# succinctlabs/sp1

Measured on AMD Instinct MI355X. Metric: RISC-V cycles proved/sec (core shard prove): whole ShardProof of a full core shard of the reference's `fibonacci` guest, see config, higher is better.
Workload: dtype u32 (KoalaBear Montgomery words, exact integer arithmetic)

## Files before the change

### __graft_entry__.py

```python
import os
import subprocess
import sys

ROOT = os.path.dirname(os.path.abspath(__file__))
CSRC = os.path.join(ROOT, "sp1_amd", "csrc")
LIB = os.path.join(ROOT, "sp1_amd", "lib", "libsp1hip.so")
HIP_SOURCES = ["runtime.hip", "merkle.hip", "ntt.hip", "ntt_fast.hip", "basefold.hip", "prover.hip", "stacked.hip", "zerocheck.hip", "zc_compile.cpp", "jagged.hip", "gkr.hip", "shard.hip", "staging.hip", "tracegen.hip", "tracegen_global.hip", "tracegen_riscv.hip", "tracegen_riscv_mem.hip", "tracegen_riscv_core.hip", "tracegen_riscv_sys.hip", "tracegen_rv64_partition.hip", "tracegen_lookup.hip", "tracegen_keccak.hip", "tracegen_weierstrass.hip", "host_par.hip", "pool.hip", "babybear.hip", "p2_host.cpp", "gkr_host.cpp", "rv64_exec.cpp", "outer.hip", "outer_host.cpp", "outer_basefold.hip", "outer_jagged.hip"]


def _stale(target, deps):
    if not os.path.exists(target):
        return True
    t = os.path.getmtime(target)
    return any(os.path.getmtime(d) > t for d in deps if os.path.exists(d))


def build_hip(force=False):
    from concurrent.futures import ThreadPoolExecutor
    srcs = [os.path.join(CSRC, s) for s in HIP_SOURCES if os.path.exists(os.path.join(CSRC, s))]
    headers = [os.path.join(CSRC, f) for f in os.listdir(CSRC) if f.endswith((".hpp", ".inc"))]
    headers.append(os.path.join(ROOT, "include", "sp1hip.h"))
    objdir = os.path.join(ROOT, "sp1_amd", "lib", "obj")
    os.makedirs(objdir, exist_ok=True)
    flags = ["--offload-arch=gfx950", "-O3", "-std=c++17", "-fPIC", "-Wall", "-Wno-unused-function", "-Wno-pass-failed"]
    extra = {"zerocheck.hip": ["-mllvm", "-pragma-unroll-threshold=1000000"]}
    objs, jobs = [], []
    for src in srcs:
        obj = os.path.join(objdir, os.path.basename(src)[:-4] + ".o")
        objs.append(obj)
        if force or _stale(obj, [src] + headers):
            jobs.append(["hipcc"] + (flags if src.endswith(".hip") else flags[1:]) + extra.get(os.path.basename(src), []) + ["-c", src, "-o", obj])
    if jobs:
        with ThreadPoolExecutor(max_workers=min(len(jobs), os.cpu_count() or 1)) as ex:
            list(ex.map(lambda cmd: subprocess.check_call(cmd, cwd=ROOT), jobs))
    if jobs or force or _stale(LIB, objs):
        subprocess.check_call(["hipcc", "--offload-arch=gfx950", "-shared", "-fPIC"] + objs + ["-lpthread", "-ldl", "-o", LIB], cwd=ROOT)
    build_native_tests()
    return LIB


def build_oracle(force=False):
    sys.path.insert(0, os.path.join(ROOT, "oracle"))
    import pyoracle
    return pyoracle.build(force)


def build_native_tests():
    exes = []
    for name, deps in (("rs_finish_stress", ["round_sync.hpp", "kb31.hpp", "common.hpp"]),
                       ("bn254_ops", ["bn254.hpp", "outer_poseidon2_rc.inc"]),
                       ("kb31_ops", ["kb31.hpp"]),
                       ("bb31_ops", ["bb31.hpp", "bb_poseidon2_rc.inc"]),
                       ("secp_rows", ["fp256.hpp", "tg_field_op.hpp", "kb31.hpp"]),
                       ("riscv_rows", ["tg_riscv_rows.hpp", "kb31.hpp", os.path.join(ROOT, "include", "sp1hip.h")]),
                       ("riscv_mem_rows", ["tg_riscv_mem_rows.hpp", "tg_riscv_rows.hpp", "kb31.hpp", os.path.join(ROOT, "include", "sp1hip.h")]),
                       ("riscv_core_rows", ["tg_riscv_core_rows.hpp", "tg_riscv_rows.hpp", "kb31.hpp", os.path.join(ROOT, "include", "sp1hip.h")]),
                       ("riscv_sys_rows", ["tg_riscv_sys_rows.hpp", "tg_rv64_partition.hpp", "tg_riscv_core_rows.hpp", "tg_riscv_rows.hpp", "kb31.hpp",
                                           os.path.join(ROOT, "include", "sp1hip.h")]),
                       ("lookup_counts", ["tg_lookup_counts.hpp", "kb31.hpp", os.path.join(ROOT, "include", "sp1hip.h")]),
                       ("septic_ops", ["septic.hpp", "poseidon2.hpp", "kb_poseidon2_rc.inc", "kb31.hpp"])):
        src = os.path.join(ROOT, "tests", "native", name + ".hip")
        exe = src[:-4]
        if not os.path.exists(src):
            continue
        if _stale(exe, [src] + [os.path.join(CSRC, d) for d in deps]):
            subprocess.check_call(["hipcc", "--offload-arch=gfx950", "-O3", "-std=c++17", "-I" + CSRC, "-I" + os.path.join(ROOT, "include"),
                                   src, "-ldl", "-o", exe], cwd=ROOT)
        exes.append(exe)
    return exes


def build():
    build_hip()
    build_oracle()
    sys.path.insert(0, ROOT)
    import sp1_amd
    lib = sp1_amd._lib.load()
    assert lib.sp1hip_version().startswith(b"sp1hip")
    subprocess.check_call([sys.executable, os.path.join(ROOT, "rust", "gen_sys.py")], stdout=subprocess.DEVNULL)


def smoke():
    sys.path.insert(0, ROOT)
    sys.path.insert(0, os.path.join(ROOT, "oracle"))
    import numpy as np
    import torch
    assert torch.cuda.is_available(), "smoke() needs a GPU"
    torch.cuda.set_device(0)
    import pyoracle as orc
    from sp1_amd import api

    lg_n, widths = 12, [16, 8]
    mles = [orc.random_felts((1 << lg_n, w), seed=7 + i) for i, w in enumerate(widths)]
    o_round = orc.CommittedRound(mles, 2)
    o_ch = orc.Challenger()
    o_ch.observe(o_round.commit)
    o_point = o_ch.sample_point(lg_n)
    o_claims = [orc.eval_mle(m, o_point) for m in mles]
    o_blob = orc.basefold_prove(o_point, [o_round], [o_claims], o_ch, 2, 16, 8)
    prover = api.BasefoldProver(2, 16, 8)
    d_mles = [api.ColMajor.from_row_major_host(m) for m in mles]
    commit, pd = prover.commit_mles(d_mles)
    assert np.array_equal(commit, o_round.commit), "commitment mismatch vs oracle"
    ch = api.DuplexChallenger()
    ch.observe(commit)
    point = ch.sample_point(lg_n)
    assert np.array_equal(point, o_point)
    claims = prover.evaluate_mles(d_mles, point)
    assert np.array_equal(claims, np.concatenate(o_claims)), "evaluation claims mismatch vs oracle"
    blob = prover.prove_trusted_mle_evaluations(point, [pd], claims, ch)
    assert blob == o_blob, "BaseFold proof bytes differ from the oracle"
    v_ch = orc.Challenger()
    v_ch.observe(commit)
    v_ch.sample_point(lg_n)
    assert orc.basefold_verify([commit], point, [claims], blob, v_ch, 2, 16, 8) == 0
    sys.path.insert(0, os.path.join(ROOT, "tests"))
    from shard_chips import make_shard_chips, preprocessed_round
    L, lsh, batch = 4, 3, 3
    chips, publics = make_shard_chips(5, 24, True, 3)
    o_prep = preprocessed_round(chips, L, lsh, batch, 1)
    jp = api.JaggedProver(L, lsh, batch, 1)
    dev = [(a, i, api.ColMajor.from_row_major_host(m) if m.shape[0] else None,
            api.ColMajor.from_row_major_host(p) if p is not None and p.shape[0] else None) for a, i, m, p in chips]
    g_commit, g_prep = jp.commit_multilinears([d[3] for d in dev if d[3] is not None])
    o_ch, g_ch = orc.Challenger(), api.DuplexChallenger()
    o_ch.observe(o_prep.commit)
    g_ch.observe(g_commit)
    v_ch = o_ch.clone()
    want = orc.shard_prove(chips, publics, o_prep, L, lsh, batch, o_ch, 1, 5, 4)
    got = api.prove_shard(dev, publics, g_prep, L, lsh, batch, g_ch, 1, 5, 4)
    assert got == want, "shard proof bytes differ from the oracle"
    assert orc.shard_verify(chips, g_commit, got, L, lsh, v_ch, 1, 5, 4) == 0
    sys.path.insert(0, os.path.join(ROOT, "bench"))
    import core_real
    from sp1_amd.machines import riscv_trace as RT
    counts = {"Add": 3, "Addi": 5, "Sub": 2, "Bitwise": 3, "Lt": 3, "Mul": 3, "ShiftLeft": 3, "ShiftRight": 3, "UType": 8,
              "LoadWord": 3, "LoadDouble": 3, "StoreWord": 3, "StoreDouble": 3, "Branch": 5, "Jal": 2, "Jalr": 2}
    machine, tabs, rpub = RT.generate(counts, K=2, seed=11, device="cuda")
    rpv = RT.to_monty_np(rpub)
    host = [(a, i, RT.to_monty_np(tabs[a.name][1]), RT.to_monty_np(tabs[a.name][0]) if tabs[a.name][0] is not None else None)
            for a, i in machine]
    rdev = [(a, i, core_real.to_col_major(tabs[a.name][1]), core_real.to_col_major(tabs[a.name][0]) if tabs[a.name][0] is not None else None)
            for a, i in machine]
    L, lsh, batch = 17, 12, 8
    r_prep = orc.JaggedRound([c[3] for c in host if c[3] is not None], L, lsh, batch, 1)
    rg_commit, rg_prep = api.JaggedProver(L, lsh, batch, 1).commit_multilinears([d[3] for d in rdev if d[3] is not None])
    assert np.array_equal(rg_commit, r_prep.commit), "RISC-V machine: preprocessed commitment differs from the oracle"
    o_ch, g_ch = orc.Challenger(), api.DuplexChallenger()
    o_ch.observe(r_prep.commit)
    g_ch.observe(rg_commit)
    orc.set_gkr_sparse(True)
    try:
        r_want = orc.shard_prove(host, rpv, r_prep, L, lsh, batch, o_ch, 1, 5, 4)
    finally:
        orc.set_gkr_sparse(False)
    r_got = api.prove_shard(rdev, rpv, rg_prep, L, lsh, batch, g_ch, 1, 5, 4)
    assert r_got == r_want, "RISC-V machine: shard proof bytes differ from the oracle"
    from sp1_amd.machines import riscv_more_trace as MT
    kmachine, ktabs, kpub = MT.precompile_shard(2, seed=3, device="cuda")
    khost = [(a, i, RT.to_monty_np(ktabs[a.name][1].cpu()), RT.to_monty_np(ktabs[a.name][0].cpu()) if ktabs[a.name][0] is not None else None)
             for a, i in kmachine]
    kdev = [(a, i, core_real.to_col_major(ktabs[a.name][1]), core_real.to_col_major(ktabs[a.name][0]) if ktabs[a.name][0] is not None else None)
            for a, i in kmachine]
    k_prep = orc.JaggedRound([c[3] for c in khost if c[3] is not None], L, lsh, batch, 1)
    kg_commit, kg_prep = api.JaggedProver(L, lsh, batch, 1).commit_multilinears([d[3] for d in kdev if d[3] is not None])
    o_ch, g_ch = orc.Challenger(), api.DuplexChallenger()
    o_ch.observe(k_prep.commit)
    g_ch.observe(kg_commit)
    publics = RT.to_monty_np(kpub.cpu())
    orc.set_gkr_sparse(True)
    try:
        k_want = orc.shard_prove(khost, publics, k_prep, L, lsh, batch, o_ch, 1, 5, 4)
    finally:
        orc.set_gkr_sparse(False)
    k_got = api.prove_shard(kdev, publics, kg_prep, L, lsh, batch, g_ch, 1, 5, 4)
    assert k_got == k_want, "Keccak precompile shard: proof bytes differ from the oracle"
    import struct
    from sp1_amd.machines import riscv_exec as RX
    ex = RX.Executor(RX.guest_file("fibonacci.elf"), stdin=[struct.pack("<Q", 20)])
    shard = ex.run_shard(1 << 20)
    assert shard.halted and shard.exit_code == 0, "the fibonacci guest did not halt cleanly"
    fmachine, ftabs, fpub = RX.shard_tables(ex, shard, device="cuda")
    fhost = [(a, i, RT.to_monty_np(ftabs[a.name][1]), RT.to_monty_np(ftabs[a.name][0]) if ftabs[a.name][0] is not None else None)
             for a, i in fmachine]
    fdev = [(a, i, core_real.to_col_major(ftabs[a.name][1]), core_real.to_col_major(ftabs[a.name][0]) if ftabs[a.name][0] is not None else None)
            for a, i in fmachine]
    fpv = RT.to_monty_np(fpub)
    f_prep = orc.JaggedRound([c[3] for c in fhost if c[3] is not None], L, lsh, batch, 1)
    fg_commit, fg_prep = api.JaggedProver(L, lsh, batch, 1).commit_multilinears([d[3] for d in fdev if d[3] is not None])
    o_ch, g_ch = orc.Challenger(), api.DuplexChallenger()
    o_ch.observe(f_prep.commit)
    g_ch.observe(fg_commit)
    orc.set_gkr_sparse(True)
    try:
        f_want = orc.shard_prove(fhost, fpv, f_prep, L, lsh, batch, o_ch, 1, 5, 4)
    finally:
        orc.set_gkr_sparse(False)
    f_got = api.prove_shard(fdev, fpv, fg_prep, L, lsh, batch, g_ch, 1, 5, 4)
    assert f_got == f_want, "fibonacci guest: shard proof bytes differ from the oracle"
    from sp1_amd.machines import public_values as PVM
    assert frozenset(a.name for a, _ in fmachine) in RT.chip_clusters(), "fibonacci guest: the shard is not a shape cluster"
    v_ch = orc.Challenger()
    v_ch.observe(f_prep.commit)
    shapes = [(a, i, np.zeros((0, a.main_width), np.uint32), np.zeros((0, a.prep_width), np.uint32) if a.prep_width else None) for a, i in fmachine]
    assert orc.shard_verify(shapes, fg_commit, f_got, L, lsh, v_ch, 1, 5, 4, pv_program=PVM.verifier_program()) == 0, \
        "fibonacci guest: the pinned verifier rejects the shard proof"
    torch.cuda.synchronize()
    print("smoke OK: commitment, claims, %d-byte BaseFold proof, %d-byte whole shard proof, a %d-byte proof of the rv64im machine "
          "(%d chips), a %d-byte proof of a Keccak precompile shard and a %d-byte proof of the reference's fibonacci guest "
          "(%d cycles) bit-identical to the oracle"
          % (len(blob), len(got), len(r_got), len(machine), len(k_got), len(f_got), shard.cycles))


if __name__ == "__main__":
    build()
    if len(sys.argv) > 1 and sys.argv[1] == "smoke":
        smoke()
```

### sp1_amd/csrc/gkr.hip

```cpp
#include <algorithm>
#include <array>
#include <chrono>
#include <cstring>
#include <optional>
#include <string>
#include <vector>

#include "device_ctx.hpp"
#include "host_par.hpp"

namespace sp1hip {
bool gkr_host_simd_available();
void gkr_host_round_sums(const uint32_t* tab, size_t stride, const uint32_t* eq, size_t eq_stride, size_t real_pairs, uint32_t out[6][4]);
void gkr_host_round_fold(const uint32_t* tab, uint32_t* out, size_t stride, size_t real_pairs, const uint32_t alpha[4]);
}
#include "round_sync.hpp"
#include "tensor_table.hpp"
#include "ext_host.hpp"
#include "gkr_kernels.hpp"

namespace sp1hip {

void challenger_observe(sp1hip_challenger_t* ch, uint32_t x);
kb::Ext challenger_sample_ext(sp1hip_challenger_t* ch);
void challenger_restore(sp1hip_challenger_t* dst, const sp1hip_challenger_t* src);

namespace gkr {

using namespace ext_host;

using Poly4 = std::array<Ext, 4>;
Ext poly_eval(const Poly4& c, const Ext& x) { return ((c[3] * x + c[2]) * x + c[1]) * x + c[0]; }

Poly4 interpolate4(const Ext (&xs)[4], const Ext (&ys)[4]) {
    Poly4 res{kb::ext_zero(), kb::ext_zero(), kb::ext_zero(), kb::ext_zero()};
    Ext num[4][4], den[4];
    bool live[4];
    for (int i = 0; i < 4; i++) {
        live[i] = !kb::ext_eq(ys[i], kb::ext_zero());
        if (!live[i]) continue;
        den[i] = kb::ext_one();
        Ext cur[4] = {ys[i], kb::ext_zero(), kb::ext_zero(), kb::ext_zero()};
        int deg = 0;
        for (int j = 0; j < 4; j++) {
            if (j == i) continue;
            den[i] = den[i] * (xs[i] - xs[j]);
            Ext nxt[4] = {kb::ext_zero(), kb::ext_zero(), kb::ext_zero(), kb::ext_zero()};
            for (int k = 0; k <= deg; k++) { nxt[k + 1] = nxt[k + 1] + cur[k]; nxt[k] = nxt[k] - cur[k] * xs[j]; }
            deg++;
            for (int k = 0; k < 4; k++) cur[k] = nxt[k];
        }
        for (int k = 0; k < 4; k++) num[i][k] = cur[k];
    }
    Ext prefix[4], running = kb::ext_one();
    for (int i = 0; i < 4; i++) if (live[i]) { prefix[i] = running; running = running * den[i]; }
    Ext inv_all = kb::ext_inv(running);
    for (int i = 3; i >= 0; i--) {
        if (!live[i]) continue;
        const Ext inv = inv_all * prefix[i];
        inv_all = inv_all * den[i];
        for (int k = 0; k < 4; k++) res[k] = res[k] + num[i][k] * inv;
    }
    return res;
}

struct Bytes {
    std::vector<uint8_t> b;
    void u64(uint64_t v) { for (int i = 0; i < 8; i++) b.push_back((uint8_t)(v >> (8 * i))); }
    void felt(uint32_t m) { const uint32_t v = kb::from_monty(m); for (int i = 0; i < 4; i++) b.push_back((uint8_t)(v >> (8 * i))); }
    void ext(const Ext& e) { for (int k = 0; k < 4; k++) felt(e.c[k]); }
};

void observe_ext(sp1hip_challenger_t* ch, const Ext& e) { for (int k = 0; k < 4; k++) challenger_observe(ch, e.c[k]); }

struct ChipInfo {
    std::string name;
    uint32_t rows, k, main_w, prep_w, int0;
    const uint32_t* d_main;
    const uint32_t* d_prep;
};

constexpr uint32_t MAX_TILES = 512;
uint32_t tiles_for(uint64_t threads) { return (uint32_t)std::min<uint64_t>(std::max<uint64_t>((threads + 255) / 256, 1), MAX_TILES); }

struct ParsedInt { uint32_t is_send, kind; std::vector<uint32_t> mult; std::vector<std::vector<uint32_t>> values; };
struct RoundOut { Ext n0, n1, d0, d1; std::vector<Poly4> polys; Ext claimed_sum, eval; std::vector<Ext> point; };
struct PassShape { int fv, sv; bool first; uint32_t tiles, tile_size, total_slots; size_t flat_off; bool flat; };

struct GkrTimer {
    enum Part { ROWS, INT, LAYER_HEAD, WAIT, HOST, LAUNCH, SKIP };
    using Clock = std::chrono::steady_clock;
    bool on = false;
    Clock::time_point last, clk[2];
    double part_ms[7] = {};
    int waits = 0;
    static double ms(Clock::time_point a, Clock::time_point b) { return std::chrono::duration<double, std::milli>(b - a).count(); }
    void start() { static const bool env = env_flag("SP1HIP_GKR_DEBUG", false); on = env; last = Clock::now(); }
    void mark(const char* what) {
        if (!on) return;
        const auto now = Clock::now();
        fprintf(stderr, "[sp1hip gkr] %-28s %8.3f ms\n", what, ms(last, now));
        last = now;
    }
    void lap(Part p) {
        if (!on) return;
        const auto now = Clock::now();
        part_ms[p] += ms(clk[p >= WAIT], now);
        clk[p >= WAIT] = now;
        waits += p == WAIT;
    }
    void report_layers() {
        if (!on) return;
        fprintf(stderr, "[sp1hip gkr]   of which row-variable rounds %.3f ms, interaction-variable rounds (host) %.3f ms\n", part_ms[ROWS], part_ms[INT]);
        fprintf(stderr, "[sp1hip gkr]   %d hand-overs inside the layers: waiting for the sums %.3f ms, closed forms + transcript %.3f ms, launch calls %.3f ms\n",
                waits, part_ms[WAIT], part_ms[HOST], part_ms[LAUNCH]);
    }
};

struct Levels {
    int L = 0;
    uint32_t K = 0;
    std::vector<uint32_t> h;
    std::vector<size_t> entries;
    std::vector<std::vector<size_t>> off;
    std::vector<DeviceBuf> N, D;
    uint32_t rows_at(uint32_t i, int l) const { return (uint32_t)(((uint64_t)h[i] + (((uint64_t)1 << (L - l)) - 1)) >> (L - l)); }
    void* n_ptr(int l, uint32_t i) const { return (char*)N[l].p + off[l][i] * (l == L ? 4 : 16); }
    Ext* d_ptr(int l, uint32_t i) const { return D[l].ext() + off[l][i]; }
    int alloc(int L_, std::vector<uint32_t> rows_of_interaction, hipStream_t s) {
        L = L_; h = std::move(rows_of_interaction); K = (uint32_t)h.size();
        entries.assign(L + 2, 0);
        off.assign(L + 1, std::vector<size_t>(K + 1, 0));
        for (int l = 1; l <= L; l++) {
            for (uint32_t i = 0; i < K; i++) off[l][i + 1] = off[l][i] + rows_at(i, l);
            entries[l] = off[l][K];
        }
        N = std::vector<DeviceBuf>(L + 1); D = std::vector<DeviceBuf>(L + 1);
        for (int l = 1; l <= L; l++) {
            SP1HIP_TRY(N[l].alloc(std::max<size_t>(entries[l], 1) * (l == L ? 4 : 16), s));
            SP1HIP_TRY(D[l].alloc(std::max<size_t>(entries[l], 1) * 16, s));
        }
        return SP1HIP_SUCCESS;
    }
};

struct PassPlan {
    std::vector<PassShape> shapes;
    std::vector<PassDesc> all_descs;
    std::vector<uint16_t> flat_index;
};
size_t count_passes(int L) { size_t n = 0; for (int v = 1; v <= L - 1; v++) n += (size_t)(v + 1) / 2 + 1; return n; }

void plan_passes(const Levels& lv, uint32_t flat_max_slots, Ext* const (&scratch)[2], Ext* host_rows, PassPlan& plan) {
    const uint32_t K = lv.K;
    auto scratch_ptr = [&](int b, uint32_t i, int which, const std::vector<size_t>& so) -> Ext* { return scratch[b] + 4 * so[i] + (size_t)which * (so[i + 1] - so[i]); };
    constexpr uint32_t TARGET_TILES = 2048;
    plan.all_descs.reserve(count_passes(lv.L) * K);
    std::vector<uint32_t> rows_in(K);
    std::vector<size_t> so_prev, so_next;
    for (int v = 1; v <= lv.L - 1; v++) {
        for (uint32_t i = 0; i < K; i++) rows_in[i] = (lv.rows_at(i, v + 1) + 1) / 2;
        int cur = 0, t = v, fv = 0, pass = 0;
        for (;;) {
            const int sv = std::min(2, t - fv);
            const bool first = pass <= 1;
            if (fv > 0) { so_next.assign(K + 1, 0); for (uint32_t i = 0; i < K; i++) so_next[i + 1] = so_next[i] + ((rows_in[i] + (1u << fv) - 1) >> fv); }
            uint64_t total_slots = 0;
            auto slots_of = [&](uint32_t rin) -> uint32_t { const uint32_t ro = (rin + (1u << fv) - 1) >> fv; return ((ro + (1u << sv) - 1) >> sv) << sv; };
            for (uint32_t i = 0; i < K; i++) total_slots += slots_of(rows_in[i]);
            const bool flat = total_slots <= flat_max_slots && K <= 65536;
            const uint32_t tile_size = flat ? 1u : (uint32_t)std::max<uint64_t>(256, ((total_slots + TARGET_TILES - 1) / TARGET_TILES + 255) / 256 * 256);
            const size_t flat_off = plan.flat_index.size();
            plan.all_descs.resize(plan.all_descs.size() + K);
            PassDesc* out = plan.all_descs.data() + plan.all_descs.size() - K;
            uint32_t tile0 = 0;
            for (uint32_t i = 0; i < K; i++) {
                PassDesc& d = out[i];
                d = PassDesc{};
                d.rows_in = rows_in[i]; d.eq_int_index = i;
                if (first) { d.src[0] = lv.n_ptr(v + 1, i); d.src[1] = lv.d_ptr(v + 1, i); d.rows_x = lv.rows_at(i, v + 1); }
                else for (int w = 0; w < 4; w++) d.src[w] = scratch_ptr(cur ^ 1, i, w, so_prev);
                if (fv > 0) for (int w = 0; w < 4; w++)
                    d.dst[w] = (sv == 0 && host_rows) ? host_rows + 4 * so_next[i] + (size_t)w * (so_next[i + 1] - so_next[i]) : scratch_ptr(cur, i, w, so_next);
                d.tile0 = tile0;
                const uint32_t n_tiles = (slots_of(rows_in[i]) + tile_size - 1) / tile_size;
                if (flat) plan.flat_index.insert(plan.flat_index.end(), n_tiles, (uint16_t)i);
                tile0 += n_tiles;
            }
            if (flat) plan.shapes.push_back(PassShape{fv, sv, first, std::max<uint32_t>((tile0 + 255) / 256, 1), tile_size, tile0, flat_off, true});
            else plan.shapes.push_back(PassShape{fv, sv, first, std::max<uint32_t>(tile0, 1), tile_size, tile0, 0, false});
            if (fv > 0) { for (uint32_t i = 0; i < K; i++) rows_in[i] = (rows_in[i] + (1u << fv) - 1) >> fv; so_prev = so_next; cur ^= 1; }
            t -= fv;
            pass++;
            if (sv == 0) break;
            fv = sv;
        }
    }
    if (plan.flat_index.empty()) plan.flat_index.push_back(0);
    plan.flat_index.resize((plan.flat_index.size() + 1) / 2 * 2);
}

struct Consts { const Ext one = kb::ext_one(), zero = kb::ext_zero(), inv8 = kb::ext_inv(ext_c(8)), inv2 = kb::ext_inv(ext_c(2)), four = ext_c(4); };

struct LayerRounds {
    sp1hip_challenger_t* ch;
    RoundOut ro;
    std::vector<Ext> alphas;
    Ext claim;
    Ext finish_round(const Poly4& poly, const Ext& pt, Ext& eq_factor) {
        ro.polys.push_back(poly);
        for (auto& c : poly) observe_ext(ch, c);
        const Ext a = challenger_sample_ext(ch), one = kb::ext_one();
        alphas.push_back(a);
        claim = poly_eval(poly, a);
        eq_factor = eq_factor * (pt * a + (one - pt) * (one - a));
        return a;
    }
};

Poly4 eq_times_quadratic(const Ext& scale, const Ext& pt, const Ext (&q)[3]) {
    const Ext e0 = scale * (kb::ext_one() - pt), e1 = scale * (pt + pt - kb::ext_one());
    return Poly4{e0 * q[0], e0 * q[1] + e1 * q[0], e0 * q[2] + e1 * q[1], e1 * q[2]};
}
void quadratic(const Ext& g0, const Ext& g1, const Ext& gi, Ext (&q)[3]) { q[0] = g0; q[1] = g1 - g0 - gi; q[2] = gi; }
Ext eval_quadratic(const Ext (&q)[3], const Ext& x) { return (q[2] * x + q[1]) * x + q[0]; }

void row_rounds_closed_form(int sv, const Ext (&S)[10], const std::vector<Ext>& row_point, int t, Ext& PA, LayerRounds& lr, Ext& a0, Ext& a1) {
    const Ext one = kb::ext_one(), pt_a = row_point[t - 1];
    if (sv == 2) {
        const Ext pt_b = row_point[t - 2];
        const Ext corr = one - S[9];
        Ext c0[3], c1[3], ci[3];
        quadratic(S[0] + corr, S[1] + corr, S[4], c0);
        quadratic(S[2] + corr, S[3] + corr, S[5], c1);
        quadratic(S[6], S[7], S[8], ci);
        Ext h[3];
        for (int k = 0; k < 3; k++) h[k] = c0[k] + pt_b * (c1[k] - c0[k]);
        a0 = lr.finish_round(eq_times_quadratic(PA, pt_a, h), pt_a, PA);
        const Ext g0 = eval_quadratic(c0, a0), g1 = eval_quadratic(c1, a0), gi = eval_quadratic(ci, a0);
        Ext gy[3];
        quadratic(g0, g1, gi, gy);
        a1 = lr.finish_round(eq_times_quadratic(PA, pt_b, gy), pt_b, PA);
    } else {
        const Ext corr = one - S[3];
        Ext h[3];
        quadratic(S[0] + corr, S[1] + corr, S[2], h);
        a0 = lr.finish_round(eq_times_quadratic(PA, pt_a, h), pt_a, PA);
        a1 = kb::ext_zero();
    }
}

constexpr size_t plane_stride(size_t n) { return ((n + 15) / 16) * 16 + 16; }

struct EqTabs {
    std::vector<std::vector<Ext>> tabs;
    std::vector<std::vector<uint32_t>> soa;
    void build(const std::vector<Ext>& int_point, bool simd) {
        const int niv = (int)int_point.size();
        tabs.assign(niv + 1, {}); soa.assign(niv + 1, {});
        tabs[0] = {kb::ext_one()};
        for (int m = 0; m < niv; m++) {
            const std::vector<Ext>& ev = tabs[m];
            std::vector<Ext>& nx = tabs[m + 1];
            nx.resize(ev.size() * 2);
            const Ext x = int_point[m];
            for (size_t i = 0; i < ev.size(); i++) { const Ext pr = ev[i] * x; nx[2 * i] = ev[i] - pr; nx[2 * i + 1] = pr; }
        }
        if (!simd) return;
        for (int m = 1; m <= niv; m++) {
            const size_t es = plane_stride((size_t)1 << m);
            soa[m].assign(4 * es, 0u);
            for (size_t i = 0; i < tabs[m].size(); i++)
                for (int k = 0; k < 4; k++) soa[m][(size_t)k * es + i] = tabs[m][i].c[k];
        }
    }
};

struct alignas(64) RoundSums { Ext x0, y0, xh, yh, e0, es; };

struct PlaneTables {
    const EqTabs& eq;
    const size_t stride;
    std::vector<uint32_t> soa[2];
    int side = 0;
    PlaneTables(const EqTabs& eq_, uint32_t W) : eq(eq_), stride(plane_stride(W)) {
        for (int b = 0; b < 2; b++) {
            soa[b].assign(16 * stride, 0u);
            for (int w = 1; w < 4; w += 2) std::fill_n(soa[b].begin() + (size_t)(4 * w) * stride, stride, kb::R1);
        }
    }
    void set_row(uint32_t i, const Ext* row) { for (int q = 0; q < 16; q++) soa[0][(size_t)q * stride + i] = row[q / 4].c[q % 4]; }
    RoundSums sums(int m, size_t real_pairs) const {
        uint32_t o6[6][4];
        gkr_host_round_sums(soa[side].data(), stride, eq.soa[m].data(), plane_stride((size_t)1 << m), real_pairs, o6);
        RoundSums t;
        Ext* dstp[6] = {&t.x0, &t.y0, &t.xh, &t.yh, &t.e0, &t.es};
        for (int q = 0; q < 6; q++) memcpy(dstp[q]->c, o6[q], 16);
        return t;
    }
    void fold(size_t real_pairs, size_t half, const Ext& alpha) {
        gkr_host_round_fold(soa[side].data(), soa[side ^ 1].data(), stride, real_pairs, alpha.c);
        if (real_pairs < half)
            for (int w = 0; w < 4; w++)
                for (int k = 0; k < 4; k++) soa[side ^ 1][(size_t)(4 * w + k) * stride + real_pairs] = (w & 1) && k == 0 ? kb::R1 : 0u;
        side ^= 1;
    }
    void first_row(Ext (&f)[4]) const { for (int q = 0; q < 16; q++) f[q / 4].c[q % 4] = soa[side][(size_t)q * stride]; }
};

struct ScalarTables {
    const EqTabs& eq;
    HostPar::Scope& par;
    std::vector<Ext> tab[2][4];
    int side = 0;
    ScalarTables(const EqTabs& eq_, HostPar::Scope& par_, uint32_t W) : eq(eq_), par(par_) {
        for (int w = 0; w < 4; w++) { tab[0][w].assign(W, (w & 1) ? kb::ext_one() : kb::ext_zero()); tab[1][w].resize(W / 2 + 1); }
    }
    void set_row(uint32_t i, const Ext* row) { for (int w = 0; w < 4; w++) tab[0][w][i] = row[w]; }
    RoundSums sums(int m, size_t real_pairs) const {
        const std::vector<Ext>& eqi = eq.tabs[m];
        const Ext *n0 = tab[side][0].data(), *d0 = tab[side][1].data(), *n1 = tab[side][2].data(), *d1 = tab[side][3].data();
        RoundSums parts[HostPar::Scope::MAX_THREADS];
        const int nparts = par.threads();
        for (int q = 0; q < nparts; q++) parts[q] = RoundSums{kb::ext_zero(), kb::ext_zero(), kb::ext_zero(), kb::ext_zero(), kb::ext_zero(), kb::ext_zero()};
        par.run(real_pairs, 24, [&](int part, size_t kb0, size_t ke) {
            RoundSums acc = parts[part];
            for (size_t k = kb0; k < ke; k++) {
                const size_t a = 2 * k, b = 2 * k + 1;
                acc.x0 = acc.x0 + eqi[a] * (d0[a] * n1[a] + d1[a] * n0[a]);
                acc.y0 = acc.y0 + eqi[a] * (d0[a] * d1[a]);
                const Ext sn0 = n0[a] + n0[b], sn1 = n1[a] + n1[b], sd0 = d0[a] + d0[b], sd1 = d1[a] + d1[b];
                const Ext es = eqi[a] + eqi[b];
                acc.xh = acc.xh + es * (sd0 * sn1 + sd1 * sn0);
                acc.yh = acc.yh + es * (sd0 * sd1);
                acc.e0 = acc.e0 + eqi[a];
                acc.es = acc.es + es;
            }
            parts[part] = acc;
        });
        RoundSums t = parts[0];
        for (int q = 1; q < nparts; q++) {
            t.x0 = t.x0 + parts[q].x0; t.y0 = t.y0 + parts[q].y0; t.xh = t.xh + parts[q].xh; t.yh = t.yh + parts[q].yh;
            t.e0 = t.e0 + parts[q].e0; t.es = t.es + parts[q].es;
        }
        return t;
    }
    void fold(size_t real_pairs, size_t half, const Ext& alpha) {
        const Ext *n0 = tab[side][0].data(), *d0 = tab[side][1].data(), *n1 = tab[side][2].data(), *d1 = tab[side][3].data();
        Ext *o0 = tab[side ^ 1][0].data(), *o1 = tab[side ^ 1][1].data(), *o2 = tab[side ^ 1][2].data(), *o3 = tab[side ^ 1][3].data();
        par.run(real_pairs, 48, [&](int, size_t kb0, size_t ke) {
            for (size_t k = kb0; k < ke; k++) {
                o0[k] = n0[2 * k] + alpha * (n0[2 * k + 1] - n0[2 * k]); o1[k] = d0[2 * k] + alpha * (d0[2 * k + 1] - d0[2 * k]);
                o2[k] = n1[2 * k] + alpha * (n1[2 * k + 1] - n1[2 * k]); o3[k] = d1[2 * k] + alpha * (d1[2 * k + 1] - d1[2 * k]);
            }
        });
        if (real_pairs < half) { o0[real_pairs] = kb::ext_zero(); o1[real_pairs] = kb::ext_one(); o2[real_pairs] = kb::ext_zero(); o3[real_pairs] = kb::ext_one(); }
        side ^= 1;
    }
    void first_row(Ext (&f)[4]) const { for (int w = 0; w < 4; w++) f[w] = tab[side][w][0]; }
};

template <class Tables>
void interaction_rounds(Tables& tb, size_t real, const std::vector<Ext>& int_point, const Ext& lambda, const Ext& PA, const Consts& k, LayerRounds& lr) {
    const int niv = (int)int_point.size();
    Ext eq_scale = k.one;
    for (int j = 0; j < niv; j++) {
        const size_t half = ((size_t)1 << (niv - j)) / 2, real_pairs = (real + 1) / 2;
        const RoundSums t = tb.sums(niv - j, real_pairs);
        const Ext pt = int_point[niv - 1 - j];
        const Ext s0 = lambda * t.x0 + t.y0 + ((k.one - pt) - t.e0);
        const Ext sh = lambda * t.xh + t.yh + (k.one - t.es) * k.four;
        const Ext PAe = PA * eq_scale;
        const Ext p0 = PAe * s0, ph = PAe * sh * k.inv8;
        const Ext xs[4] = {k.zero, k.one, k.inv2, (k.one - pt) * kb::ext_inv(k.one - (pt + pt))};
        const Ext ys[4] = {p0, lr.claim - p0, ph, k.zero};
        tb.fold(real_pairs, half, lr.finish_round(interpolate4(xs, ys), pt, eq_scale));
        real = real_pairs;
    }
    Ext f[4];
    tb.first_row(f);
    lr.ro.n0 = f[0]; lr.ro.d0 = f[1]; lr.ro.n1 = f[2]; lr.ro.d1 = f[3];
}

void interaction_rounds_host(bool simd, HostPar::Scope& par, const EqTabs& eq, uint32_t W, const std::vector<size_t>& so, const Ext* rows,
                             const std::vector<Ext>& int_point, const Ext& lambda, const Ext& PA, const Consts& k, LayerRounds& lr, GkrTimer& timer) {
    auto run = [&](auto tb) {
        const uint32_t K = (uint32_t)so.size() - 1;
        for (uint32_t i = 0; i < K; i++) if (so[i + 1] != so[i]) tb.set_row(i, rows + 4 * so[i]);
        timer.lap(GkrTimer::ROWS);
        interaction_rounds(tb, K, int_point, lambda, PA, k, lr);
        timer.lap(GkrTimer::INT);
    };
    if (simd) run(PlaneTables(eq, W)); else run(ScalarTables(eq, par, W));
}

#define SP1HIP_GKR_REQUIRE(cond, msg) \
    do { if (!(cond)) { sp1hip::set_error("sp1hip_logup_gkr_prove: %s", msg); return SP1HIP_ERROR_INVALID_ARGUMENT; } } while (0)

struct GkrProver {
    const sp1hip_gkr_chip_t* const chips;
    const int n_chips, L;
    sp1hip_challenger_t* const challenger;
    uint8_t* const h_proof;
    size_t* const proof_len;
    const sp1hip_stream_t stream;
    const hipStream_t s;

    GkrTimer timer;
    const Consts k;
    std::vector<ChipInfo> info;
    std::vector<ParsedInt> progs;
    size_t max_arity = 0, total_cols = 0, need = 0;
    uint32_t K = 0, W = 0;
    int niv = 0;
    struct Cloned { sp1hip_challenger_t* c = nullptr; ~Cloned() { sp1hip_challenger_free(c); } } clone;
    sp1hip_challenger_t* ch = nullptr;
    uint32_t witness = 0, flat_max_slots = 0;
    Ext alpha;
    std::vector<Ext> betas;
    std::vector<uint32_t> int_chip;
    Levels lv;
    size_t n_passes_total = 0;
    hipStream_t side = nullptr;
    hipEvent_t* side_ev = nullptr;
    DeviceBuf d_all, d_flat;
    PinnedStage side_stage, stage;
    DeviceBuf d_progs, d_betas, d_descs;
    std::vector<uint32_t> flat;
    std::vector<IntDesc> descs;
    DeviceBuf d_trans, d_trans2;
    Mailbox mb;
    DeviceBuf d_eq_int, d_T, d_TL, d_partials, scratch[2];
    bool direct_final = false, simd = false;
    PassPlan plan;
    std::vector<Ext> out_n, out_d, eval_point;
    Ext num_eval, den_eval;
    size_t launch_idx = 0;
    RoundSyncHost rsync;
    std::optional<HostPar::Scope> par;
    std::vector<RoundOut> rounds;
    std::vector<Ext> trace_point, openings;

    int parse_programs() {
        info.resize(n_chips);
        for (int c = 0; c < n_chips; c++) {
            const sp1hip_gkr_chip_t& ci = chips[c];
            SP1HIP_GKR_REQUIRE(ci.name && ci.interactions, "null chip field");
            SP1HIP_GKR_REQUIRE(ci.real_rows <= ((uint64_t)1 << L), "chip taller than 2^max_log_row_count");
            SP1HIP_GKR_REQUIRE(ci.real_rows == 0 || ci.main_width == 0 || ci.d_main, "null main trace");
            SP1HIP_GKR_REQUIRE(ci.real_rows == 0 || ci.prep_width == 0 || ci.d_prep, "null preprocessed trace");
            if (c) SP1HIP_GKR_REQUIRE(strcmp(chips[c - 1].name, ci.name) < 0, "chips must be sorted by name (BTreeSet order)");
            info[c] = ChipInfo{ci.name, (uint32_t)ci.real_rows, 0, ci.main_width, ci.prep_width, (uint32_t)progs.size(), ci.d_main, ci.d_prep};
            const uint32_t* p = ci.interactions;
            const uint32_t* end = p + ci.n_words;
            SP1HIP_GKR_REQUIRE(ci.n_words >= 1, "empty interaction program");
            const uint32_t ni = *p++;
            info[c].k = ni;
            auto vcol = [&](std::vector<uint32_t>& out) -> bool {
                if (p + 2 > end) return false;
                const uint32_t nt = p[0];
                if (p[1] >= kb::P || p + 2 + 3 * (size_t)nt > end) return false;
                out.push_back(nt);
                out.push_back(kb::to_monty(p[1]));
                p += 2;
                for (uint32_t t = 0; t < nt; t++, p += 3) {
                    if (p[0] > 1 || p[2] >= kb::P) return false;
                    if (p[1] >= (p[0] ? ci.main_width : ci.prep_width)) return false;
                    out.push_back(p[0]); out.push_back(p[1]); out.push_back(kb::to_monty(p[2]));
                }
                return true;
            };
            for (uint32_t i = 0; i < ni; i++) {
                SP1HIP_GKR_REQUIRE(p + 3 <= end, "truncated interaction program");
                const uint32_t nv = p[2];
                SP1HIP_GKR_REQUIRE(p[0] <= 1 && p[1] < kb::P && nv < 4096, "bad interaction header");
                ParsedInt pi{p[0], p[1], {}, std::vector<std::vector<uint32_t>>(nv)};
                p += 3;
                SP1HIP_GKR_REQUIRE(vcol(pi.mult), "bad multiplicity column");
                for (uint32_t j = 0; j < nv; j++) SP1HIP_GKR_REQUIRE(vcol(pi.values[j]), "bad value column (index or weight out of range)");
                max_arity = std::max<size_t>(max_arity, nv + 1);
                progs.push_back(std::move(pi));
            }
            SP1HIP_GKR_REQUIRE(p == end, "trailing words in interaction program");
            total_cols += (size_t)ci.main_width + ci.prep_width;
        }
        K = (uint32_t)progs.size();
        SP1HIP_GKR_REQUIRE(K >= 1, "no interactions in the shard");
        niv = log2_ceil(K);
        W = 1u << niv;
        return SP1HIP_SUCCESS;
    }

    size_t proof_size() const {
        size_t n = 2 * (8 + (size_t)2 * W * 16 + 24) + 8;
        for (int v = 1; v <= L - 1; v++) n += 64 + 8 + (size_t)(niv + v) * (8 + 64) + 16 + 8 + (size_t)(niv + v) * 16 + 16;
        n += 8 + (size_t)L * 16 + 8;
        for (int c = 0; c < n_chips; c++) {
            n += 8 + info[c].name.size() + 8 + (size_t)info[c].main_w * 16 + 16 + 1;
            if (info[c].prep_w) n += 8 + (size_t)info[c].prep_w * 16 + 16;
        }
        return n + 4;
    }

    int transcript_head() {
        SP1HIP_TRY(sp1hip_challenger_clone(challenger, &clone.c));
        ch = clone.c;
        SP1HIP_TRY(sp1hip_challenger_grind(ch, 12, &witness, stream));
        alpha = challenger_sample_ext(ch);
        std::vector<Ext> beta_seed(log2_ceil(max_arity));
        for (auto& b : beta_seed) b = challenger_sample_ext(ch);
        (void)challenger_sample_ext(ch);
        betas = partial_lagrange_host(beta_seed);
        return SP1HIP_SUCCESS;
    }

    int alloc_levels_and_plan_buffers() {
        int_chip.resize(K);
        std::vector<uint32_t> rows(K);
        for (int c = 0; c < n_chips; c++) for (uint32_t i = 0; i < info[c].k; i++) { int_chip[info[c].int0 + i] = c; rows[info[c].int0 + i] = info[c].rows; }
        SP1HIP_TRY(lv.alloc(L, std::move(rows), s));
        timer.mark("parse + level buffers");
        flat_max_slots = (uint32_t)env_uint("SP1HIP_GKR_FLAT_SLOTS", 65536);
        n_passes_total = count_passes(L);
        SP1HIP_TRY(aux_stream_for(s, 2, &side, &side_ev));
        SP1HIP_TRY(d_all.alloc(std::max<size_t>(n_passes_total * K, 1) * sizeof(PassDesc), side));
        SP1HIP_TRY(d_flat.alloc((n_passes_total * (size_t)flat_max_slots + 4) * sizeof(uint16_t), side));
        SP1HIP_TRY(side_stage.init(side));
        return stage.init(s);
    }

    int build_first_layer_and_tree() {
        std::vector<size_t> poff(K);
        for (uint32_t i = 0; i < K; i++) {
            poff[i] = flat.size();
            const ParsedInt& pi = progs[i];
            Ext head = alpha + kb::ext_mul_base(betas[0], kb::to_monty(pi.kind));
            uint32_t live = 0;
            for (size_t j = 0; j < pi.values.size(); j++) {
                if (pi.values[j][0] == 0) head = head + kb::ext_mul_base(betas[1 + j], pi.values[j][1]);
                else live++;
            }
            flat.insert(flat.end(), {pi.is_send, live, head.c[0], head.c[1], head.c[2], head.c[3]});
            flat.insert(flat.end(), pi.mult.begin(), pi.mult.end());
            for (size_t j = 0; j < pi.values.size(); j++) {
                if (pi.values[j][0] == 0) continue;
                flat.push_back((uint32_t)(1 + j));
                flat.insert(flat.end(), pi.values[j].begin(), pi.values[j].end());
            }
        }
        SP1HIP_TRY(upload(d_progs, flat.data(), flat.size() * 4, s, stage));
        SP1HIP_TRY(upload(d_betas, betas.data(), betas.size() * 16, s, stage));
        uint32_t max_rows = 0;
        descs.resize(K);
        for (uint32_t i = 0; i < K; i++) {
            const ChipInfo& c = info[int_chip[i]];
            descs[i] = IntDesc{d_progs.u32() + poff[i], c.d_main, c.d_prep, c.rows, (uint32_t*)lv.n_ptr(L, i), lv.d_ptr(L, i)};
            max_rows = std::max(max_rows, c.rows);
        }
        const bool fused_tree = L >= 3 && env_flag("SP1HIP_GKR_FUSED", true);
        if (fused_tree) {
            std::vector<FirstDesc> fdescs(K);
            for (uint32_t i = 0; i < K; i++)
                fdescs[i] = FirstDesc{descs[i].prog, descs[i].main, descs[i].prep, descs[i].rows, descs[i].n_out, descs[i].d_out,
                                      (Ext*)lv.n_ptr(L - 1, i), lv.d_ptr(L - 1, i), (Ext*)lv.n_ptr(L - 2, i), lv.d_ptr(L - 2, i)};
            SP1HIP_TRY(upload(d_descs, fdescs.data(), fdescs.size() * sizeof(FirstDesc), s, stage));
            if (max_rows) {
                ScopedTimer t("gkr_first_layer", s);
                hipLaunchKernelGGL(first_layers_kernel, dim3(tiles_for((max_rows + 3) / 4), K), dim3(256), 0, s, (const FirstDesc*)d_descs.p,
                                   (const Ext*)d_betas.p);
                SP1HIP_LAUNCH_CHECK();
            }
        } else {
            SP1HIP_TRY(upload(d_descs, descs.data(), descs.size() * sizeof(IntDesc), s, stage));
            if (max_rows) {
                ScopedTimer t("gkr_first_layer", s);
                hipLaunchKernelGGL(first_layer_kernel, dim3(tiles_for(max_rows), K), dim3(256), 0, s, (const IntDesc*)d_descs.p,
                                   (const Ext*)d_betas.p);
                SP1HIP_LAUNCH_CHECK();
            }
        }
        timer.mark("first layer enqueued");
        const int top = fused_tree ? L - 2 : L;
        std::vector<Trans2Desc> t2;
        std::vector<TransDesc> t1;
        std::vector<uint32_t> t2_mr, t1_mr;
        std::vector<int> t1_level;
        int l = top;
        if (fused_tree)
            for (; l >= 3; l -= 2) {
                uint32_t mr = 0;
                for (uint32_t i = 0; i < K; i++) {
                    const uint32_t rin = lv.rows_at(i, l);
                    t2.push_back(Trans2Desc{(const Ext*)lv.n_ptr(l, i), lv.d_ptr(l, i), (Ext*)lv.n_ptr(l - 1, i), lv.d_ptr(l - 1, i), (Ext*)lv.n_ptr(l - 2, i), lv.d_ptr(l - 2, i), rin});
                    mr = std::max(mr, (rin + 3) / 4);
                }
                t2_mr.push_back(mr);
            }
        for (; l >= 2; l--) {
            uint32_t mr = 0;
            for (uint32_t i = 0; i < K; i++) {
                const uint32_t rin = lv.rows_at(i, l);
                t1.push_back(TransDesc{lv.n_ptr(l, i), lv.d_ptr(l, i), (Ext*)lv.n_ptr(l - 1, i), lv.d_ptr(l - 1, i), rin});
                mr = std::max(mr, (rin + 1) / 2);
            }
            t1_mr.push_back(mr);
            t1_level.push_back(l);
        }
        if (!t2.empty()) SP1HIP_TRY(upload(d_trans2, t2.data(), t2.size() * sizeof(Trans2Desc), s, stage));
        if (!t1.empty()) SP1HIP_TRY(upload(d_trans, t1.data(), t1.size() * sizeof(TransDesc), s, stage));
        for (size_t j = 0; j < t2_mr.size(); j++) {
            if (!t2_mr[j]) continue;
            ScopedTimer t("gkr_transition", s);
            hipLaunchKernelGGL(transition2_kernel, dim3(tiles_for(t2_mr[j]), K), dim3(256), 0, s, (const Trans2Desc*)d_trans2.p + j * K);
            SP1HIP_LAUNCH_CHECK();
        }
        for (size_t j = 0; j < t1_mr.size(); j++) {
            if (!t1_mr[j]) continue;
            const TransDesc* d_t = (const TransDesc*)d_trans.p + j * K;
            ScopedTimer t("gkr_transition", s);
            if (t1_level[j] == L) hipLaunchKernelGGL(transition_kernel<true>, dim3(tiles_for(t1_mr[j]), K), dim3(256), 0, s, d_t);
            else hipLaunchKernelGGL(transition_kernel<false>, dim3(tiles_for(t1_mr[j]), K), dim3(256), 0, s, d_t);
            SP1HIP_LAUNCH_CHECK();
        }
        timer.mark("tree enqueued");
        return SP1HIP_SUCCESS;
    }

    int plan_and_upload_passes() {
        SP1HIP_TRY(mb.init(s));
        SP1HIP_TRY(d_eq_int.alloc((size_t)W * 16, s));
        SP1HIP_TRY(d_T.alloc(((size_t)2 << std::max(L - 1, 1)) * 16, s));
        SP1HIP_TRY(d_TL.alloc(((size_t)2 << std::max(L - 1, 1)) * 16, s));
        size_t scratch_entries = 0;
        for (uint32_t i = 0; i < K; i++) scratch_entries += (lv.rows_at(i, L) + 3) / 4 + 1;
        for (int b = 0; b < 2; b++) SP1HIP_TRY(scratch[b].alloc(std::max<size_t>(scratch_entries, 1) * 64, s));
        direct_final = (size_t)K * 16 + 4 <= MAILBOX_WORDS;
        Ext* const scratch_ext[2] = {scratch[0].ext(), scratch[1].ext()};
        plan_passes(lv, flat_max_slots, scratch_ext, direct_final ? reinterpret_cast<Ext*>(mb.h_slot + 4) : nullptr, plan);
        {
            uint32_t max_tiles = 1;
            for (auto& sh : plan.shapes) max_tiles = std::max(max_tiles, sh.tiles);
            SP1HIP_TRY(d_partials.alloc((size_t)max_tiles * 160, s));
        }
        timer.mark("pass descriptors planned");
        SP1HIP_GKR_REQUIRE(plan.all_descs.size() == n_passes_total * K, "internal error: pass count");
        SP1HIP_TRY(side_stage.upload(d_all.p, plan.all_descs.data(), plan.all_descs.size() * sizeof(PassDesc)));
        SP1HIP_GKR_REQUIRE(plan.flat_index.size() * sizeof(uint16_t) <= d_flat.n, "internal error: flat index size");
        SP1HIP_TRY(side_stage.upload(d_flat.p, plan.flat_index.data(), plan.flat_index.size() * sizeof(uint16_t)));
        SP1HIP_HIP(hipEventRecord(side_ev[1], side));
        SP1HIP_HIP(hipStreamWaitEvent(s, side_ev[1], 0));
        timer.mark("pass descriptors uploaded");
        return SP1HIP_SUCCESS;
    }

    int fetch_circuit_output() {
        out_n.assign(2 * (size_t)W, kb::ext_zero()); out_d.assign(2 * (size_t)W, kb::ext_one());
        std::vector<Ext> hn(std::max<size_t>(lv.entries[1], 1)), hd(std::max<size_t>(lv.entries[1], 1));
        if (L >= 2) {
            SP1HIP_TRY(mb.fetch(lv.N[1].p, lv.entries[1] * 4, hn.data()));
        } else {
            std::vector<uint32_t> hb(std::max<size_t>(lv.entries[1], 1));
            SP1HIP_TRY(mb.fetch(lv.N[1].p, lv.entries[1], hb.data()));
            for (size_t e = 0; e < lv.entries[1]; e++) hn[e] = kb::ext_from_base(hb[e]);
        }
        SP1HIP_TRY(mb.fetch(lv.D[1].p, lv.entries[1] * 4, hd.data()));
        for (uint32_t i = 0; i < K; i++)
            for (uint32_t r = 0; r < lv.rows_at(i, 1); r++) { out_n[2 * i + r] = hn[lv.off[1][i] + r]; out_d[2 * i + r] = hd[lv.off[1][i] + r]; }
        timer.mark("circuit output fetched");
        challenger_observe(ch, kb::to_monty(2 * W));
        for (auto& e : out_n) observe_ext(ch, e);
        challenger_observe(ch, kb::to_monty(2 * W));
        for (auto& e : out_d) observe_ext(ch, e);
        eval_point.resize(niv + 1);
        for (auto& z : eval_point) z = challenger_sample_ext(ch);
        num_eval = eval_mle_host(out_n, eval_point); den_eval = eval_mle_host(out_d, eval_point);
        return SP1HIP_SUCCESS;
    }

#define SP1HIP_GKR_PASS(FV, SV, F, NB, FL) hipLaunchKernelGGL((gkr_pass<FV, SV, F, NB, FL>), dim3(shape.tiles), dim3(256), 0, s, d_descs, (const Ext*)d_eq_int.p, Tp, TLp, c0, c1, d_partials.u32(), rs, publish_rows ? mb.seq + 1 : rsync.seq, K, shape.tile_size, fa)
#define SP1HIP_GKR_PASS_FL(FV, SV, F, NB) do { if (shape.flat) SP1HIP_GKR_PASS(FV, SV, F, NB, true); else SP1HIP_GKR_PASS(FV, SV, F, NB, false); } while (0)
#define SP1HIP_GKR_PASS_SRC(FV, SV) do { if (nbase) SP1HIP_GKR_PASS_FL(FV, SV, true, true); else if (shape.first) SP1HIP_GKR_PASS_FL(FV, SV, true, false); else SP1HIP_GKR_PASS_FL(FV, SV, false, false); } while (0)
    int launch_pass(size_t idx, int v, int t_after, const Ext& c0, const Ext& c1) {
        const PassShape shape = plan.shapes[idx];
        const PassDesc* d_descs = (const PassDesc*)d_all.p + idx * K;
        const int fv = shape.fv, sv = shape.sv;
        const FlatArgs fa{(const uint16_t*)d_flat.p + shape.flat_off, shape.total_slots};
        const bool nbase = shape.first && v + 1 == L;
        const bool publish_rows = sv == 0 && direct_final;
        if (publish_rows) { rsync.pending = true; mb.pending = true; }
        const RoundSync rs = sv > 0 ? rsync.next() : publish_rows ? RoundSync{rsync.d_counter, (volatile uint32_t*)mb.h_slot} : RoundSync{};
        const Ext* Tp = sv > 0 ? d_T.ext() + (((size_t)1 << (t_after - sv)) - 1) : (const Ext*)nullptr;
        const Ext* TLp = sv > 0 ? d_TL.ext() + (((size_t)1 << (t_after - sv)) - 1) : (const Ext*)nullptr;
        ScopedTimer tm(fv == 0 ? "gkr_pass_sum" : sv == 0 ? "gkr_pass_fold" : "gkr_pass_fold_sum", s);
        if (fv == 0 && sv == 2) { if (nbase) SP1HIP_GKR_PASS_FL(0, 2, true, true); else SP1HIP_GKR_PASS_FL(0, 2, true, false); }
        else if (fv == 0 && sv == 1) { if (nbase) SP1HIP_GKR_PASS_FL(0, 1, true, true); else SP1HIP_GKR_PASS_FL(0, 1, true, false); }
        else if (fv == 2 && sv == 2) SP1HIP_GKR_PASS_SRC(2, 2);
        else if (fv == 2 && sv == 1) SP1HIP_GKR_PASS_SRC(2, 1);
        else if (fv == 2 && sv == 0) SP1HIP_GKR_PASS_SRC(2, 0);
        else if (fv == 1 && sv == 0) SP1HIP_GKR_PASS_SRC(1, 0);
        else { set_error("internal error: GKR pass shape (%d, %d)", fv, sv); return SP1HIP_ERROR_RUNTIME; }
        SP1HIP_LAUNCH_CHECK();
        return SP1HIP_SUCCESS;
    }
#undef SP1HIP_GKR_PASS_SRC
#undef SP1HIP_GKR_PASS_FL
#undef SP1HIP_GKR_PASS

    int prove_layer(int v) {
        timer.lap(GkrTimer::LAYER_HEAD);
        const Ext lambda = challenger_sample_ext(ch);
        LayerRounds lr{ch, {}, {}, num_eval * lambda + den_eval};
        lr.ro.claimed_sum = lr.claim;
        const std::vector<Ext> int_point(eval_point.begin(), eval_point.begin() + niv), row_point(eval_point.begin() + niv, eval_point.end());
        SP1HIP_GKR_REQUIRE(niv <= 32 && v <= 32, "point too long");
        {
            PointArg pi{}, pa{};
            for (int j = 0; j < niv; j++) pi.c[j] = int_point[j];
            for (int j = 0; j < v; j++) pa.c[j] = row_point[j];
            const uint32_t full_blocks = (W + 255) / 256, prefix_blocks = ((2u << v) + 255) / 256;
            hipLaunchKernelGGL(eq_layer_tables_kernel, dim3(full_blocks + prefix_blocks), dim3(256), 0, s, pi, niv, d_eq_int.ext(), full_blocks, pa, v,
                               lambda, d_T.ext(), d_TL.ext());
            SP1HIP_LAUNCH_CHECK();
        }
        EqTabs eq_tabs;
        Ext PA = k.one;
        Ext a0 = k.zero, a1 = k.zero;
        int t = v;
        for (bool first_pass = true;; first_pass = false) {
            const size_t idx = launch_idx++;
            const int fv = plan.shapes[idx].fv, sv = plan.shapes[idx].sv;
            t -= fv;
            if (!simd && t == sv) par->wake();
            timer.lap(first_pass ? GkrTimer::SKIP : GkrTimer::HOST);
            SP1HIP_TRY(launch_pass(idx, v, t, a0, a1));
            timer.lap(GkrTimer::LAUNCH);
            if (first_pass) eq_tabs.build(int_point, simd);
            if (sv == 0) break;
            const int ns = sv == 2 ? 10 : 4;
            uint32_t h_sums[40];
            timer.lap(GkrTimer::SKIP);
            SP1HIP_TRY(rsync.wait(h_sums, 4 * ns));
            timer.lap(GkrTimer::WAIT);
            Ext S[10];
            memcpy(S, h_sums, 16 * (size_t)ns);
            row_rounds_closed_form(sv, S, row_point, t, PA, lr, a0, a1);
        }
        std::vector<size_t> so(K + 1, 0);
        for (uint32_t i = 0; i < K; i++) so[i + 1] = so[i] + (lv.rows_at(i, v + 1) ? 1 : 0);
        const size_t final_rows_total = so[K];
        const int cur = (int)((((v + 1) / 2)) & 1) ^ 1;
        std::vector<Ext> host(std::max<size_t>(final_rows_total, 1) * 4);
        if (direct_final) { SP1HIP_TRY(mb.wait_next(host.data(), final_rows_total * 16, 4)); rsync.pending = false; }
        else SP1HIP_TRY(mb.fetch(scratch[cur].p, final_rows_total * 16, host.data()));
        interaction_rounds_host(simd, *par, eq_tabs, W, so, host.data(), int_point, lambda, PA, k, lr, timer);
        RoundOut& ro = lr.ro;
        ro.eval = lr.claim;
        ro.point.assign(lr.alphas.rbegin(), lr.alphas.rend());
        observe_ext(ch, ro.n0); observe_ext(ch, ro.n1); observe_ext(ch, ro.d0); observe_ext(ch, ro.d1);
        eval_point = ro.point;
        const Ext lc = challenger_sample_ext(ch);
        num_eval = ro.n0 + (ro.n1 - ro.n0) * lc;
        den_eval = ro.d0 + (ro.d1 - ro.d0) * lc;
        eval_point.push_back(lc);
        rounds.push_back(std::move(ro));
        par->park();
        return SP1HIP_SUCCESS;
    }

    int prove_layers() {
        SP1HIP_TRY(rsync.init(s));
        simd = gkr_host_simd_available();
        par.emplace();
        par->park();
        for (int v = 1; v <= L - 1; v++) SP1HIP_TRY(prove_layer(v));
        timer.report_layers();
        timer.mark("all layers");
        return SP1HIP_SUCCESS;
    }

    int open_traces() {
        trace_point.assign(eval_point.end() - L, eval_point.end());
        openings.assign(std::max<size_t>(total_cols, 1), kb::ext_zero());
        if (!total_cols) return SP1HIP_SUCCESS;
        DeviceBuf d_eq, d_od, d_part, d_res;
        SP1HIP_TRY(d_eq.alloc(((size_t)16) << L, s));
        SP1HIP_TRY(sp1hip_partial_lagrange(reinterpret_cast<const sp1hip_ext_t*>(trace_point.data()), L, d_eq.u32(), stream));
        std::vector<OpenDesc> od;
        uint32_t out0 = 0, max_rows_open = 0;
        for (int c = 0; c < n_chips; c++) {
            for (uint32_t g = 0; g < info[c].main_w; g += OPEN_COLS) od.push_back(OpenDesc{info[c].d_main, info[c].rows, info[c].main_w, g, out0 + g});
            out0 += info[c].main_w;
            for (uint32_t g = 0; g < info[c].prep_w; g += OPEN_COLS) od.push_back(OpenDesc{info[c].d_prep, info[c].rows, info[c].prep_w, g, out0 + g});
            out0 += info[c].prep_w;
            max_rows_open = std::max(max_rows_open, info[c].rows);
        }
        const uint32_t chunks = std::max<uint32_t>((max_rows_open + OPEN_ROWS - 1) / OPEN_ROWS, 1);
        SP1HIP_TRY(upload(d_od, od.data(), od.size() * sizeof(OpenDesc), s, stage));
        SP1HIP_TRY(d_part.alloc((size_t)chunks * total_cols * 16, s));
        SP1HIP_TRY(d_res.alloc(total_cols * 16, s));
        SP1HIP_HIP(hipMemsetAsync(d_part.p, 0, (size_t)chunks * total_cols * 16, s));
        ScopedTimer t("gkr_openings", s);
        hipLaunchKernelGGL(open_columns_kernel, dim3((uint32_t)od.size(), chunks), dim3(256), 0, s, (const OpenDesc*)d_od.p, d_eq.u32(),
                           1u << L, d_part.u32(), (uint32_t)total_cols);
        SP1HIP_LAUNCH_CHECK();
        hipLaunchKernelGGL(open_sum_kernel, dim3(((uint32_t)total_cols * 4 + 63) / 64), dim3(256), 0, s, d_part.u32(), chunks,
                           (uint32_t)total_cols * 4, d_res.u32());
        SP1HIP_LAUNCH_CHECK();
        return mb.fetch(d_res.p, total_cols * 4, openings.data());
    }

    void observe_openings() {
        challenger_observe(ch, kb::to_monty((uint32_t)n_chips));
        size_t o = 0;
        for (int c = 0; c < n_chips; c++) {
            const Ext* main = openings.data() + o;
            const Ext* prep = main + info[c].main_w;
            if (info[c].prep_w) {
                challenger_observe(ch, kb::to_monty(info[c].prep_w));
                for (uint32_t j = 0; j < info[c].prep_w; j++) observe_ext(ch, prep[j]);
            }
            challenger_observe(ch, kb::to_monty(info[c].main_w));
            for (uint32_t j = 0; j < info[c].main_w; j++) observe_ext(ch, main[j]);
            o += info[c].main_w + info[c].prep_w;
        }
        timer.mark("openings");
    }

    int write_proof() {
        Bytes w;
        for (const std::vector<Ext>* vv : {&out_n, &out_d}) {
            w.u64(vv->size());
            for (auto& e : *vv) w.ext(e);
            w.u64(2); w.u64(vv->size()); w.u64(1);
        }
        w.u64(rounds.size());
        for (auto& r : rounds) {
            w.ext(r.n0); w.ext(r.n1); w.ext(r.d0); w.ext(r.d1);
            w.u64(r.polys.size());
            for (auto& p : r.polys) { w.u64(4); for (auto& c : p) w.ext(c); }
            w.ext(r.claimed_sum);
            w.u64(r.point.size());
            for (auto& x : r.point) w.ext(x);
            w.ext(r.eval);
        }
        w.u64(trace_point.size());
        for (auto& x : trace_point) w.ext(x);
        w.u64(n_chips);
        size_t o = 0;
        for (int c = 0; c < n_chips; c++) {
            w.u64(info[c].name.size());
            for (char chr : info[c].name) w.b.push_back((uint8_t)chr);
            w.u64(info[c].main_w);
            for (uint32_t j = 0; j < info[c].main_w; j++) w.ext(openings[o + j]);
            w.u64(1); w.u64(info[c].main_w);
            w.b.push_back(info[c].prep_w ? 1 : 0);
            if (info[c].prep_w) {
                w.u64(info[c].prep_w);
                for (uint32_t j = 0; j < info[c].prep_w; j++) w.ext(openings[o + info[c].main_w + j]);
                w.u64(1); w.u64(info[c].prep_w);
            }
            o += info[c].main_w + info[c].prep_w;
        }
        w.felt(witness);
        if (w.b.size() != need) {
            set_error("internal error: GKR proof size %zu != expected %zu", w.b.size(), need);
            return SP1HIP_ERROR_RUNTIME;
        }
        memcpy(h_proof, w.b.data(), w.b.size());
        *proof_len = w.b.size();
        return SP1HIP_SUCCESS;
    }

    int prove() {
        timer.start();
        SP1HIP_TRY(parse_programs());
        need = proof_size();
        if (!h_proof || *proof_len < need) {
            *proof_len = need;
            set_error("sp1hip_logup_gkr_prove: proof buffer too small, need %zu bytes", need);
            return SP1HIP_ERROR_BUFFER_TOO_SMALL;
        }
        const DeviceCtx* ctx;
        SP1HIP_TRY(get_device_ctx(&ctx));
        SP1HIP_TRY(transcript_head());
        SP1HIP_TRY(alloc_levels_and_plan_buffers());
        SP1HIP_TRY(build_first_layer_and_tree());
        SP1HIP_TRY(plan_and_upload_passes());
        SP1HIP_TRY(fetch_circuit_output());
        SP1HIP_TRY(prove_layers());
        SP1HIP_TRY(open_traces());
        observe_openings();
        SP1HIP_TRY(write_proof());
        challenger_restore(challenger, ch);
        return SP1HIP_SUCCESS;
    }
};
#undef SP1HIP_GKR_REQUIRE
}
}

using namespace sp1hip;

extern "C" int sp1hip_logup_gkr_prove(const sp1hip_gkr_chip_t* chips, int n_chips, int max_log_row_count, sp1hip_challenger_t* challenger,
                                      uint8_t* h_proof, size_t* proof_len, sp1hip_stream_t stream) {
    SP1HIP_REQUIRE(chips && n_chips > 0 && challenger && proof_len, "bad argument");
    SP1HIP_REQUIRE(max_log_row_count >= 1 && max_log_row_count <= 30, "max_log_row_count out of range");
    gkr::GkrProver p{chips, n_chips, max_log_row_count, challenger, h_proof, proof_len, stream, S(stream)};
    return p.prove();
}
```

### sp1_amd/csrc/gkr_kernels.hpp

```cpp
#pragma once
#include "device_ctx.hpp"
#include "round_sync.hpp"

namespace sp1hip {
namespace gkr {

using Ext = kb::Ext;

__device__ __forceinline__ Ext ld_ext(const Ext* p, uint32_t i) {
    const q4_t v = gptr(reinterpret_cast<const q4_t*>(p))[i];
    return Ext{{v.x, v.y, v.z, v.w}};
}
__device__ __forceinline__ void st_ext(Ext* p, uint32_t i, const Ext& e) {
    const q4_t v = {e.c[0], e.c[1], e.c[2], e.c[3]};
    gptr(reinterpret_cast<q4_t*>(p))[i] = v;
}

__device__ __forceinline__ void st_ext_host(Ext* p, uint32_t i, const Ext& e) {
    uint32_t* w = reinterpret_cast<uint32_t*>(p + i);
#pragma unroll
    for (int k = 0; k < 4; k++) __hip_atomic_store(w + k, e.c[k], __ATOMIC_RELAXED, __HIP_MEMORY_SCOPE_SYSTEM);
}

__device__ __forceinline__ uint32_t wave_sum(uint32_t v) {
#pragma unroll
    for (int off = 32; off >= 1; off >>= 1) v = kb::add(v, __shfl_down(v, off, 64));
    return v;
}
template <int NS>
__device__ __forceinline__ void block_reduce_store(const Ext (&acc)[NS], uint32_t* out) {
    __shared__ uint32_t sm[4][4 * NS];
    const int lane = threadIdx.x & 63, wave = threadIdx.x >> 6;
#pragma unroll
    for (int s = 0; s < NS; s++)
#pragma unroll
        for (int k = 0; k < 4; k++) {
            const uint32_t w = wave_sum(acc[s].c[k]);
            if (lane == 0) sm[wave][4 * s + k] = w;
        }
    __syncthreads();
    if (threadIdx.x < 4 * NS) {
        uint32_t a = 0;
        for (int i = 0; i < 4; i++) a = kb::add(a, sm[i][threadIdx.x]);
        out[threadIdx.x] = a;
    }
}
template <int NS>
__global__ __launch_bounds__(256) void reduce_partials(const uint32_t* __restrict__ partials, uint32_t n, uint32_t* out) {
    Ext acc[NS];
#pragma unroll
    for (int s = 0; s < NS; s++) acc[s] = kb::ext_zero();
    for (uint32_t i = threadIdx.x; i < n; i += 256)
#pragma unroll
        for (int s = 0; s < NS; s++) {
            const uint32_t* q = partials + ((size_t)i * NS + s) * 4;
            acc[s] = kb::ext_add(acc[s], Ext{{q[0], q[1], q[2], q[3]}});
        }
    block_reduce_store<NS>(acc, out);
}

__device__ __forceinline__ uint32_t level_pos(uint32_t e, uint32_t len) {
    return (e | 511u) < len ? ((e & ~511u) | ((e & 7u) << 6) | ((e >> 3) & 63u)) : e;
}

struct IntDesc {
    const uint32_t* prog;
    const uint32_t* main;
    const uint32_t* prep;
    uint32_t rows;
    uint32_t* n_out;
    Ext* d_out;
};

typedef const uint32_t __attribute__((address_space(4)))* prog_words_t;
__device__ __forceinline__ uint32_t vcol_apply(prog_words_t& p, const IntDesc& d, uint32_t r) {
    const uint32_t nt = p[0];
    uint32_t acc = p[1];
    p += 2;
    for (uint32_t t = 0; t < nt; t++, p += 3) {
        const uint32_t* col = (p[0] ? d.main : d.prep) + (size_t)p[1] * d.rows;
        const uint32_t v = gptr(col)[r], wgt = p[2];
        acc = kb::add(acc, wgt == kb::R1 ? v : kb::mul(v, wgt));
    }
    return acc;
}

__global__ __launch_bounds__(256) void first_layer_kernel(const IntDesc* __restrict__ descs, const Ext* __restrict__ betas) {
    const IntDesc d = descs[blockIdx.y];
    for (uint32_t r = blockIdx.x * blockDim.x + threadIdx.x; r < d.rows; r += gridDim.x * blockDim.x) {
        prog_words_t p = (prog_words_t)(uintptr_t)d.prog;
        const bool is_send = p[0] != 0;
        const uint32_t nv = p[1];
        Ext den{{p[2], p[3], p[4], p[5]}};
        p += 6;
        uint32_t m = vcol_apply(p, d, r);
        if (!is_send) m = kb::sub(0u, m);
        for (uint32_t j = 0; j < nv; j++) {
            const uint32_t bi = *p++;
            den = kb::ext_add(den, kb::ext_mul_base(ld_ext(betas, bi), vcol_apply(p, d, r)));
        }
        const uint32_t rp = level_pos(r, d.rows);
        gptr(d.n_out)[rp] = m;
        st_ext(d.d_out, rp, den);
    }
}

struct TransDesc {
    const void* n_in;
    const Ext* d_in;
    Ext* n_out;
    Ext* d_out;
    uint32_t rows_in;
};

template <bool NBASE>
__device__ __forceinline__ Ext load_n(const void* p, uint32_t i) {
    if (NBASE) return kb::ext_from_base(gptr((const uint32_t*)p)[i]);
    return ld_ext((const Ext*)p, i);
}

template <bool NBASE>
__global__ __launch_bounds__(256) void transition_kernel(const TransDesc* __restrict__ descs) {
    const TransDesc d = descs[blockIdx.y];
    const uint32_t rows_out = (d.rows_in + 1) / 2;
    for (uint32_t r = blockIdx.x * blockDim.x + threadIdx.x; r < rows_out; r += gridDim.x * blockDim.x) {
        const uint32_t ia = level_pos(2 * r, d.rows_in), ib = level_pos(2 * r + 1, d.rows_in), io = level_pos(r, rows_out);
        const Ext da = ld_ext(d.d_in, ia);
        if (2 * r + 1 < d.rows_in) {
            const Ext db = ld_ext(d.d_in, ib);
            Ext n;
            if (NBASE) {
                const uint32_t na = gptr((const uint32_t*)d.n_in)[ia], nb = gptr((const uint32_t*)d.n_in)[ib];
                n = kb::ext_add(kb::ext_mul_base(db, na), kb::ext_mul_base(da, nb));
            } else {
                n = kb::ext_add(kb::ext_mul(db, load_n<false>(d.n_in, ia)), kb::ext_mul(da, load_n<false>(d.n_in, ib)));
            }
            st_ext(d.n_out, io, n);
            st_ext(d.d_out, io, kb::ext_mul(da, db));
        } else {
            st_ext(d.n_out, io, load_n<NBASE>(d.n_in, ia));
            st_ext(d.d_out, io, da);
        }
    }
}

struct FirstDesc {
    const uint32_t* prog;
    const uint32_t* main;
    const uint32_t* prep;
    uint32_t rows;
    uint32_t* n0_out;
    Ext* d0_out;
    Ext* n1_out; Ext* d1_out;
    Ext* n2_out; Ext* d2_out;
};

__device__ __forceinline__ void vcol_apply4(prog_words_t& p, const FirstDesc& d, uint32_t q, bool vec, uint32_t (&out)[4]) {
    const uint32_t nt = p[0], c0 = p[1];
    p += 2;
#pragma unroll
    for (int j = 0; j < 4; j++) out[j] = c0;
    for (uint32_t t = 0; t < nt; t++, p += 3) {
        const uint32_t* col = (p[0] ? d.main : d.prep) + (size_t)p[1] * d.rows;
        const uint32_t wgt = p[2];
        uint32_t v[4];
        if (vec) {
            const q4_t x = gptr(reinterpret_cast<const q4_t*>(col))[q];
            v[0] = x.x; v[1] = x.y; v[2] = x.z; v[3] = x.w;
        } else {
#pragma unroll
            for (int j = 0; j < 4; j++) v[j] = 4 * q + j < d.rows ? gptr(col)[4 * q + j] : 0u;
        }
#pragma unroll
        for (int j = 0; j < 4; j++) out[j] = kb::add(out[j], wgt == kb::R1 ? v[j] : kb::mul(v[j], wgt));
    }
}

__global__ __launch_bounds__(256) void first_layers_kernel(const FirstDesc* __restrict__ descs, const Ext* __restrict__ betas) {
    const FirstDesc d = descs[blockIdx.y];
    const uint32_t quads = (d.rows + 3) / 4, rows1 = (d.rows + 1) / 2, rows2 = (rows1 + 1) / 2;
    const bool vec = (d.rows & 3u) == 0;
    for (uint32_t q = blockIdx.x * blockDim.x + threadIdx.x; q < quads; q += gridDim.x * blockDim.x) {
        prog_words_t p = (prog_words_t)(uintptr_t)d.prog;
        const bool is_send = p[0] != 0;
        const uint32_t nv = p[1];
        const Ext head{{p[2], p[3], p[4], p[5]}};
        p += 6;
        uint32_t m[4], val[4];
        vcol_apply4(p, d, q, vec, m);
        Ext den[4];
#pragma unroll
        for (int j = 0; j < 4; j++) { if (!is_send) m[j] = kb::sub(0u, m[j]); den[j] = head; }
        uint64_t acc[4][4];
#pragma unroll
        for (int j = 0; j < 4; j++)
#pragma unroll
            for (int c = 0; c < 4; c++) acc[j][c] = 0;
        uint32_t pending = 0;
        for (uint32_t k = 0; k < nv; k++) {
            const uint32_t bi = *p++;
            vcol_apply4(p, d, q, vec, val);
            const Ext b = ld_ext(betas, bi);
#pragma unroll
            for (int j = 0; j < 4; j++)
#pragma unroll
                for (int c = 0; c < 4; c++) acc[j][c] += (uint64_t)b.c[c] * val[j];
            if (++pending == 4 || k + 1 == nv) {
#pragma unroll
                for (int j = 0; j < 4; j++)
#pragma unroll
                    for (int c = 0; c < 4; c++) { den[j].c[c] = kb::add(den[j].c[c], kb::monty_reduce_wide(acc[j][c])); acc[j][c] = 0; }
                pending = 0;
            }
        }
        const uint32_t live = min(4u, d.rows - 4 * q);
#pragma unroll
        for (int j = 0; j < 4; j++)
            if ((uint32_t)j < live) {
                const uint32_t rp = level_pos(4 * q + j, d.rows);
                gptr(d.n0_out)[rp] = m[j];
                st_ext(d.d0_out, rp, den[j]);
            }
        Ext n1[2], d1[2];
#pragma unroll
        for (int h = 0; h < 2; h++) {
            if ((uint32_t)(2 * h + 1) < live) {
                n1[h] = kb::ext_add(kb::ext_mul_base(den[2 * h + 1], m[2 * h]), kb::ext_mul_base(den[2 * h], m[2 * h + 1]));
                d1[h] = kb::ext_mul(den[2 * h], den[2 * h + 1]);
            } else { n1[h] = kb::ext_from_base(m[2 * h]); d1[h] = den[2 * h]; }
            if ((uint32_t)(2 * h) < live) {
                const uint32_t io = level_pos(2 * q + h, rows1);
                st_ext(d.n1_out, io, n1[h]); st_ext(d.d1_out, io, d1[h]);
            }
        }
        const uint32_t io = level_pos(q, rows2);
        if (live > 2) {
            st_ext(d.n2_out, io, kb::ext_add(kb::ext_mul(d1[1], n1[0]), kb::ext_mul(d1[0], n1[1])));
            st_ext(d.d2_out, io, kb::ext_mul(d1[0], d1[1]));
        } else { st_ext(d.n2_out, io, n1[0]); st_ext(d.d2_out, io, d1[0]); }
    }
}

struct Trans2Desc {
    const Ext* n_in; const Ext* d_in;
    Ext* n1_out; Ext* d1_out; Ext* n2_out; Ext* d2_out;
    uint32_t rows_in;
};
__global__ __launch_bounds__(256) void transition2_kernel(const Trans2Desc* __restrict__ descs) {
    const Trans2Desc d = descs[blockIdx.y];
    const uint32_t quads = (d.rows_in + 3) / 4, rows1 = (d.rows_in + 1) / 2, rows2 = (rows1 + 1) / 2;
    for (uint32_t q = blockIdx.x * blockDim.x + threadIdx.x; q < quads; q += gridDim.x * blockDim.x) {
        const uint32_t live = min(4u, d.rows_in - 4 * q);
        Ext n[4], dd[4];
#pragma unroll
        for (int j = 0; j < 4; j++)
            if ((uint32_t)j < live) { const uint32_t ip = level_pos(4 * q + j, d.rows_in); n[j] = ld_ext(d.n_in, ip); dd[j] = ld_ext(d.d_in, ip); }
        Ext n1[2], d1[2];
#pragma unroll
        for (int h = 0; h < 2; h++) {
            if ((uint32_t)(2 * h + 1) < live) {
                n1[h] = kb::ext_add(kb::ext_mul(dd[2 * h + 1], n[2 * h]), kb::ext_mul(dd[2 * h], n[2 * h + 1]));
                d1[h] = kb::ext_mul(dd[2 * h], dd[2 * h + 1]);
            } else if ((uint32_t)(2 * h) < live) { n1[h] = n[2 * h]; d1[h] = dd[2 * h]; }
            if ((uint32_t)(2 * h) < live) {
                const uint32_t io = level_pos(2 * q + h, rows1);
                st_ext(d.n1_out, io, n1[h]); st_ext(d.d1_out, io, d1[h]);
            }
        }
        const uint32_t io = level_pos(q, rows2);
        if (live > 2) {
            st_ext(d.n2_out, io, kb::ext_add(kb::ext_mul(d1[1], n1[0]), kb::ext_mul(d1[0], n1[1])));
            st_ext(d.d2_out, io, kb::ext_mul(d1[0], d1[1]));
        } else { st_ext(d.n2_out, io, n1[0]); st_ext(d.d2_out, io, d1[0]); }
    }
}

struct PointArg { Ext c[32]; };
__global__ __launch_bounds__(256) void eq_layer_tables_kernel(PointArg pi, int niv, Ext* __restrict__ eq_int, uint32_t full_blocks,
                                                              PointArg pa, int v, Ext lambda, Ext* __restrict__ T, Ext* __restrict__ TL) {
    if (blockIdx.x < full_blocks) {
        const uint32_t i = blockIdx.x * 256u + threadIdx.x;
        if (i >= (1u << niv)) return;
        Ext acc = kb::ext_one();
        for (int j = 0; j < niv; j++) {
            const bool bit = (i >> (niv - 1 - j)) & 1u;
            acc = kb::ext_mul(acc, bit ? pi.c[j] : kb::ext_sub(kb::ext_one(), pi.c[j]));
        }
        st_ext(eq_int, i, acc);
        return;
    }
    const uint32_t g = (blockIdx.x - full_blocks) * 256u + threadIdx.x + 1;
    if (g >= (2u << v)) return;
    const int t = 31 - __clz(g);
    const uint32_t i = g - (1u << t);
    Ext acc = kb::ext_one();
    for (int j = 0; j < t; j++) {
        const bool bit = (i >> (t - 1 - j)) & 1u;
        acc = kb::ext_mul(acc, bit ? pa.c[j] : kb::ext_sub(kb::ext_one(), pa.c[j]));
    }
    st_ext(T, g - 1, acc);
    st_ext(TL, g - 1, kb::ext_mul(acc, lambda));
}

struct PassDesc {
    const void* src[4];
    Ext* dst[4];
    uint32_t rows_in;
    uint32_t rows_x;
    uint32_t eq_int_index;
    uint32_t tile0;
};

__device__ __forceinline__ uint32_t find_desc(const PassDesc* __restrict__ descs, uint32_t K, uint32_t b) {
    uint32_t lo = 0, hi = K;
    while (hi - lo > 1) {
        const uint32_t mid = (lo + hi) >> 1;
        if (descs[mid].tile0 <= b) lo = mid; else hi = mid;
    }
    return lo;
}
struct Row { Ext n0, d0, n1, d1; };

__device__ __forceinline__ uint32_t folded_pos(uint32_t r, uint32_t len) {
    return (r | 255u) < len ? ((r & ~255u) | ((r & 3u) << 6) | ((r >> 2) & 63u)) : r;
}

__device__ __forceinline__ Row padding_row() { return Row{kb::ext_zero(), kb::ext_one(), kb::ext_zero(), kb::ext_one()}; }

template <bool FIRST, bool NBASE>
__device__ __forceinline__ Row load_row(const PassDesc& d, uint32_t r) {
    Row q = padding_row();
    if (r >= d.rows_in) return q;
    if (FIRST) {
        const uint32_t ea = level_pos(2 * r, d.rows_x), eb = level_pos(2 * r + 1, d.rows_x);
        q.n0 = load_n<NBASE>(d.src[0], ea);
        q.d0 = ld_ext((const Ext*)d.src[1], ea);
        if (2 * r + 1 < d.rows_x) { q.n1 = load_n<NBASE>(d.src[0], eb); q.d1 = ld_ext((const Ext*)d.src[1], eb); }
    } else {
        const uint32_t rp = folded_pos(r, d.rows_in);
        q.n0 = ld_ext((const Ext*)d.src[0], rp); q.d0 = ld_ext((const Ext*)d.src[1], rp);
        q.n1 = ld_ext((const Ext*)d.src[2], rp); q.d1 = ld_ext((const Ext*)d.src[3], rp);
    }
    return q;
}

__device__ __forceinline__ Ext lerp(const Ext& a, const Ext& b, const Ext& t) { return kb::ext_add(a, kb::ext_mul(kb::ext_sub(b, a), t)); }
__device__ __forceinline__ Row lerp_row(const Row& a, const Row& b, const Ext& t) {
    return Row{lerp(a.n0, b.n0, t), lerp(a.d0, b.d0, t), lerp(a.n1, b.n1, t), lerp(a.d1, b.d1, t)};
}
__device__ __forceinline__ Ext lerp_base(uint32_t a, uint32_t b, const Ext& t) {
    Ext e = kb::ext_mul_base(t, kb::sub(b, a));
    e.c[0] = kb::add(e.c[0], a);
    return e;
}
template <bool NBASE>
__device__ __forceinline__ Row lerp_row_in(const Row& a, const Row& b, const Ext& t) {
    if (!NBASE) return lerp_row(a, b, t);
    return Row{lerp_base(a.n0.c[0], b.n0.c[0], t), lerp(a.d0, b.d0, t), lerp_base(a.n1.c[0], b.n1.c[0], t), lerp(a.d1, b.d1, t)};
}

template <int FV, bool FIRST, bool NBASE>
__device__ __forceinline__ Row fold_row(const PassDesc& d, uint32_t ro, const Ext& a0, const Ext& a1) {
    if constexpr (FV == 0) return load_row<FIRST, NBASE>(d, ro);
    Row in[FV == 0 ? 1 : (1 << FV)];
#pragma unroll
    for (int j = 0; j < (1 << FV); j++) in[j] = load_row<FIRST, NBASE>(d, (ro << FV) + j);
    if constexpr (FV == 1) return lerp_row_in<NBASE>(in[0], in[1], a0);
    else {
        const Row lo = lerp_row_in<NBASE>(in[0], in[1], a0), hi = lerp_row_in<NBASE>(in[2], in[3], a0);
        return lerp_row(lo, hi, a1);
    }
}

template <int CTRL>
__device__ __forceinline__ Ext dpp_ext(const Ext& e) {
    return Ext{{p2::dpp_mov<CTRL>(e.c[0]), p2::dpp_mov<CTRL>(e.c[1]), p2::dpp_mov<CTRL>(e.c[2]), p2::dpp_mov<CTRL>(e.c[3])}};
}
__device__ __forceinline__ Ext sel_ext(bool c, const Ext& a, const Ext& b) {
    return Ext{{c ? a.c[0] : b.c[0], c ? a.c[1] : b.c[1], c ? a.c[2] : b.c[2], c ? a.c[3] : b.c[3]}};
}

template <int SV> struct GridAcc { Ext a[SV == 2 ? 5 : 3]; };
template <int SV>
__device__ __forceinline__ void grid_init(GridAcc<SV>& g) {
#pragma unroll
    for (int i = 0; i < (SV == 2 ? 5 : 3); i++) g.a[i] = kb::ext_zero();
}

template <int SV, bool NB>
__device__ __forceinline__ void grid_accumulate(const Row& row, const Ext& w, const Ext& wl, uint32_t j, GridAcc<SV>& g) {
    const Ext A = kb::ext_add(NB ? kb::ext_mul_base(wl, row.n0.c[0]) : kb::ext_mul(row.n0, wl), kb::ext_mul(row.d0, w));
    const Ext B = NB ? kb::ext_mul_base(wl, row.n1.c[0]) : kb::ext_mul(row.n1, wl);
    g.a[0] = kb::ext_add(g.a[0], kb::ext_add(kb::ext_mul(B, row.d0), kb::ext_mul(A, row.d1)));
    const bool lo1 = (j & 1u) == 0;
    const Ext P = sel_ext(lo1, B, A), Q = sel_ext(lo1, row.d0, row.d1), PS = sel_ext(lo1, A, B), QS = sel_ext(lo1, row.d1, row.d0);
    const Ext DP = kb::ext_sub(P, dpp_ext<p2::DPP_QUAD_SWAP1>(PS)), DQ = kb::ext_sub(Q, dpp_ext<p2::DPP_QUAD_SWAP1>(QS));
    g.a[1] = kb::ext_add(g.a[1], kb::ext_mul(DP, DQ));
    if constexpr (SV == 2) {
        const bool lo2 = (j & 2u) == 0;
        const Ext P2 = sel_ext(lo2, B, A), Q2 = sel_ext(lo2, row.d0, row.d1), PS2 = sel_ext(lo2, A, B), QS2 = sel_ext(lo2, row.d1, row.d0);
        const Ext EP = kb::ext_sub(P2, dpp_ext<p2::DPP_QUAD_SWAP2>(PS2)), EQ = kb::ext_sub(Q2, dpp_ext<p2::DPP_QUAD_SWAP2>(QS2));
        g.a[2] = kb::ext_add(g.a[2], kb::ext_mul(EP, EQ));
        const Ext FP = kb::ext_sub(DP, dpp_ext<p2::DPP_QUAD_SWAP2>(DP)), FQ = kb::ext_sub(DQ, dpp_ext<p2::DPP_QUAD_SWAP2>(DQ));
        g.a[3] = kb::ext_add(g.a[3], kb::ext_mul(FP, FQ));
    }
    if (j == 0) g.a[SV == 2 ? 4 : 2] = kb::ext_add(g.a[SV == 2 ? 4 : 2], w);
}

template <int SV> struct GridOut { static constexpr int NS = SV == 2 ? 10 : 4; };
template <int SV>
__device__ __forceinline__ void grid_split(const GridAcc<SV>& g, uint32_t j, const Ext& scale, bool use_scale, Ext (&out)[GridOut<SV>::NS]) {
    const Ext z = kb::ext_zero();
    Ext a[SV == 2 ? 5 : 3];
#pragma unroll
    for (int i = 0; i < (SV == 2 ? 5 : 3); i++) a[i] = use_scale ? kb::ext_mul(g.a[i], scale) : g.a[i];
    if constexpr (SV == 2) {
        out[0] = j == 0 ? a[0] : z; out[1] = j == 1 ? a[0] : z; out[2] = j == 2 ? a[0] : z; out[3] = j == 3 ? a[0] : z;
        out[4] = j < 2 ? a[1] : z; out[5] = j < 2 ? z : a[1];
        out[6] = (j & 1u) == 0 ? a[2] : z; out[7] = (j & 1u) == 0 ? z : a[2];
        out[8] = j < 2 ? a[3] : z;
        out[9] = a[4];
    } else {
        out[0] = j == 0 ? a[0] : z; out[1] = j == 1 ? a[0] : z;
        out[2] = a[1];
        out[3] = a[2];
    }
}

struct FlatArgs { const uint16_t* index; uint32_t total_slots; };

template <int FV, int SV, bool FIRST, bool NBASE, bool FLAT>
__global__ __launch_bounds__(256) void gkr_pass(const PassDesc* __restrict__ descs, const Ext* __restrict__ eq_int,
                                                const Ext* __restrict__ T, const Ext* __restrict__ TL, Ext a0, Ext a1,
                                                uint32_t* __restrict__ partials, RoundSync rs, uint32_t seq, uint32_t K,
                                                uint32_t tile_size, FlatArgs fa) {
    static_assert(FV + SV > 0 && FV <= 2 && SV <= 2, "a pass folds and / or sums");
    constexpr int SVS = SV == 0 ? 1 : SV;
    GridAcc<SVS> g;
    grid_init<SVS>(g);
    const uint32_t j = threadIdx.x & ((1u << SV) - 1u);
    auto do_row = [&](const PassDesc& d, uint32_t ro, bool valid, const Ext& wi, bool use_wi) {
        const uint32_t rows_out = (d.rows_in + (1u << FV) - 1u) >> FV;
        Row row = padding_row();
        if (valid && ro < rows_out) {
            row = fold_row<FV, FIRST, NBASE>(d, ro, a0, a1);
            if (FV > 0) {
                const uint32_t rq = folded_pos(ro, rows_out);
                if (SV == 0 && rs.host_slot != nullptr) {
                    st_ext_host(d.dst[0], rq, row.n0); st_ext_host(d.dst[1], rq, row.d0); st_ext_host(d.dst[2], rq, row.n1); st_ext_host(d.dst[3], rq, row.d1);
                } else {
                    st_ext(d.dst[0], rq, row.n0); st_ext(d.dst[1], rq, row.d0); st_ext(d.dst[2], rq, row.n1); st_ext(d.dst[3], rq, row.d1);
                }
            }
        }
        if constexpr (SV > 0) {
            const uint32_t cells = (rows_out + (1u << SV) - 1u) >> SV;
            const uint32_t c = ro >> SV;
            Ext w = kb::ext_zero(), wl = kb::ext_zero();
            if (valid && c < cells) {
                w = ld_ext(T, c); wl = ld_ext(TL, c);
                if (use_wi) { w = kb::ext_mul(w, wi); wl = kb::ext_mul(wl, wi); }
            }
            grid_accumulate<SVS, FIRST && NBASE && FV == 0>(row, w, wl, j, g);
        }
    };
    Ext scale = kb::ext_one();
    if (FLAT) {
        const uint32_t p = blockIdx.x * 256 + threadIdx.x;
        const bool valid = p < fa.total_slots;
        const PassDesc d = descs[valid ? fa.index[p] : 0];
        const Ext wi = SV > 0 ? ld_ext(eq_int, d.eq_int_index) : kb::ext_one();
        do_row(d, p - d.tile0, valid, wi, true);
    } else {
        const PassDesc d = descs[find_desc(descs, K, blockIdx.x)];
        const uint32_t rows_out = (d.rows_in + (1u << FV) - 1u) >> FV;
        const uint32_t slots = ((rows_out + (1u << SV) - 1u) >> SV) << SV;
        const uint32_t k0 = (blockIdx.x - d.tile0) * tile_size, k1 = min(slots, k0 + tile_size);
        for (uint32_t base = k0; base < k1; base += 256) do_row(d, base + threadIdx.x, base + threadIdx.x < k1, scale, false);
        if (SV > 0) scale = ld_ext(eq_int, d.eq_int_index);
    }
    if constexpr (SV > 0) {
        Ext out[GridOut<SVS>::NS];
        grid_split<SVS>(g, j, scale, !FLAT, out);
        rs_finish<GridOut<SVS>::NS>(out, partials, blockIdx.x, gridDim.x, rs, seq);
    } else if (rs.host_slot != nullptr) {
        asm volatile("s_waitcnt vmcnt(0)" ::: "memory");
        __syncthreads();
        if (threadIdx.x == 0 && rs_ticket_is_last_acq_rel(rs.counter, blockIdx.x, gridDim.x)) rs_publish_seq(rs.host_slot, seq);
    }
}

struct OpenDesc { const uint32_t* cols; uint32_t rows, width, col0, out0; };
constexpr int OPEN_COLS = 4, OPEN_ROWS = 16384;
__global__ __launch_bounds__(256) void open_columns_kernel(const OpenDesc* __restrict__ descs, const uint32_t* __restrict__ eq,
                                                           uint32_t eq_len, uint32_t* __restrict__ partials, uint32_t total_cols) {
    const OpenDesc d = descs[blockIdx.x];
    const uint32_t r0 = blockIdx.y * OPEN_ROWS;
    if (r0 >= d.rows) return;
    kb::DotAcc acc[OPEN_COLS];
#pragma unroll
    for (int c = 0; c < OPEN_COLS; c++) kb::dot_init(acc[c]);
    for (uint32_t r = r0 + threadIdx.x; r < r0 + OPEN_ROWS && r < d.rows; r += 256) {
        const Ext e{{eq[r], eq[eq_len + r], eq[2 * (size_t)eq_len + r], eq[3 * (size_t)eq_len + r]}};
#pragma unroll
        for (int c = 0; c < OPEN_COLS; c++)
            if (d.col0 + c < d.width) kb::dot_add(acc[c], e, gptr(d.cols)[(size_t)(d.col0 + c) * d.rows + r]);
    }
    __shared__ uint32_t sm[4][4 * OPEN_COLS];
    const int lane = threadIdx.x & 63, wave = threadIdx.x >> 6;
#pragma unroll
    for (int c = 0; c < OPEN_COLS; c++) {
        const Ext v = kb::dot_finish(acc[c]);
#pragma unroll
        for (int k = 0; k < 4; k++) {
            const uint32_t w = wave_sum(v.c[k]);
            if (lane == 0) sm[wave][4 * c + k] = w;
        }
    }
    __syncthreads();
    if (threadIdx.x < 4 * OPEN_COLS) {
        const int c = threadIdx.x / 4;
        if (d.col0 + c < d.width) {
            uint32_t a = 0;
            for (int i = 0; i < 4; i++) a = kb::add(a, sm[i][threadIdx.x]);
            partials[((size_t)blockIdx.y * total_cols + d.out0 + c) * 4 + (threadIdx.x & 3)] = a;
        }
    }
}
__global__ __launch_bounds__(256) void open_sum_kernel(const uint32_t* __restrict__ partials, uint32_t n_chunks, uint32_t n_words, uint32_t* __restrict__ out) {
    __shared__ uint32_t sm[256];
    const uint32_t jl = threadIdx.x & 63u, cl = threadIdx.x >> 6, j = blockIdx.x * 64u + jl;
    uint32_t acc = 0;
    if (j < n_words)
        for (uint32_t c = cl; c < n_chunks; c += 4) acc = kb::add(acc, partials[(size_t)c * n_words + j]);
    sm[threadIdx.x] = acc;
    __syncthreads();
    if (cl == 0 && j < n_words) out[j] = kb::add(kb::add(sm[jl], sm[64 + jl]), kb::add(sm[128 + jl], sm[192 + jl]));
}
}
}
```

### sp1_amd/csrc/round_sync.hpp

```cpp
#pragma once
#include <chrono>
#include <cstring>
#include <vector>
#include <algorithm>

#include "common.hpp"
#include "kb31.hpp"

#if defined(__HIP_DEVICE_COMPILE__) && !defined(__gfx950__) && !defined(__gfx942__)
#error "round_sync.hpp: the sc1 + vmcnt(0) hand-over is only valid on gfx942/gfx950"
#endif

namespace sp1hip {

struct RoundSync {
    uint32_t* counter;
    volatile uint32_t* host_slot;
};

constexpr uint32_t RS_GROUPS = 32, RS_GROUP_STRIDE = 64;
constexpr size_t RS_COUNTER_BYTES = (size_t)(RS_GROUPS + 1) * RS_GROUP_STRIDE * 4;
constexpr size_t RS_SLOT_WORDS = 64;

__device__ __forceinline__ bool rs_ticket_is_last(uint32_t* counter, uint32_t block_linear, uint32_t total_blocks) {
    const uint32_t g = block_linear % RS_GROUPS, members = (total_blocks - g + RS_GROUPS - 1) / RS_GROUPS;
    uint32_t* cg = counter + g * RS_GROUP_STRIDE;
    if (__hip_atomic_fetch_add(cg, 1u, __ATOMIC_RELAXED, __HIP_MEMORY_SCOPE_AGENT) != members - 1) return false;
    __hip_atomic_store(cg, 0u, __ATOMIC_RELAXED, __HIP_MEMORY_SCOPE_AGENT);
    uint32_t* c2 = counter + RS_GROUPS * RS_GROUP_STRIDE;
    const uint32_t groups = total_blocks < RS_GROUPS ? total_blocks : RS_GROUPS;
    if (__hip_atomic_fetch_add(c2, 1u, __ATOMIC_RELAXED, __HIP_MEMORY_SCOPE_AGENT) != groups - 1) return false;
    __hip_atomic_store(c2, 0u, __ATOMIC_RELAXED, __HIP_MEMORY_SCOPE_AGENT);
    return true;
}
__device__ __forceinline__ bool rs_ticket_is_last_acq_rel(uint32_t* counter, uint32_t block_linear, uint32_t total_blocks) {
    const uint32_t g = block_linear % RS_GROUPS, members = (total_blocks - g + RS_GROUPS - 1) / RS_GROUPS;
    uint32_t* cg = counter + g * RS_GROUP_STRIDE;
    if (__hip_atomic_fetch_add(cg, 1u, __ATOMIC_ACQ_REL, __HIP_MEMORY_SCOPE_AGENT) != members - 1) return false;
    __hip_atomic_store(cg, 0u, __ATOMIC_RELAXED, __HIP_MEMORY_SCOPE_AGENT);
    uint32_t* c2 = counter + RS_GROUPS * RS_GROUP_STRIDE;
    const uint32_t groups = total_blocks < RS_GROUPS ? total_blocks : RS_GROUPS;
    if (__hip_atomic_fetch_add(c2, 1u, __ATOMIC_ACQ_REL, __HIP_MEMORY_SCOPE_AGENT) != groups - 1) return false;
    __hip_atomic_store(c2, 0u, __ATOMIC_RELAXED, __HIP_MEMORY_SCOPE_AGENT);
    return true;
}
__device__ __forceinline__ void rs_publish_seq(volatile uint32_t* slot, uint32_t seq) {
    __hip_atomic_store(const_cast<uint32_t*>(slot), seq, __ATOMIC_RELEASE, __HIP_MEMORY_SCOPE_SYSTEM);
}
__device__ __forceinline__ void rs_store_partial(uint32_t* p, uint32_t v) { __hip_atomic_store(p, v, __ATOMIC_RELAXED, __HIP_MEMORY_SCOPE_AGENT); }
__device__ __forceinline__ kb::Ext rs_load_partial(const uint32_t* q) {
    kb::Ext e;
#pragma unroll
    for (int k = 0; k < 4; k++) e.c[k] = __hip_atomic_load(q + k, __ATOMIC_RELAXED, __HIP_MEMORY_SCOPE_AGENT);
    return e;
}

__device__ __forceinline__ uint32_t rs_wave_sum(uint32_t v) {
#pragma unroll
    for (int off = 32; off >= 1; off >>= 1) v = kb::add(v, __shfl_down(v, off, 64));
    return v;
}

template <int NS>
__device__ __forceinline__ void rs_finish(const kb::Ext (&acc)[NS], uint32_t* __restrict__ partials, uint32_t block_linear,
                                          uint32_t total_blocks, RoundSync rs, uint32_t seq) {
    __shared__ uint32_t sm[4][4 * NS];
    __shared__ uint32_t last_flag;
    const int lane = threadIdx.x & 63, wave = threadIdx.x >> 6;
#pragma unroll
    for (int s = 0; s < NS; s++)
#pragma unroll
        for (int k = 0; k < 4; k++) {
            const uint32_t w = rs_wave_sum(acc[s].c[k]);
            if (lane == 0) sm[wave][4 * s + k] = w;
        }
    __syncthreads();
    if (threadIdx.x < 4 * NS) {
        uint32_t a = 0;
        for (int i = 0; i < 4; i++) a = kb::add(a, sm[i][threadIdx.x]);
        rs_store_partial(&partials[(size_t)block_linear * 4 * NS + threadIdx.x], a);
    }
    asm volatile("s_waitcnt vmcnt(0)" ::: "memory");
    __syncthreads();
    if (threadIdx.x == 0) last_flag = rs_ticket_is_last(rs.counter, block_linear, total_blocks);
    __syncthreads();
    if (!last_flag) return;
    kb::Ext tot[NS];
#pragma unroll
    for (int s = 0; s < NS; s++) tot[s] = kb::ext_zero();
    for (uint32_t i = threadIdx.x; i < total_blocks; i += 256)
#pragma unroll
        for (int s = 0; s < NS; s++)
            tot[s] = kb::ext_add(tot[s], rs_load_partial(partials + ((size_t)i * NS + s) * 4));
    __syncthreads();
#pragma unroll
    for (int s = 0; s < NS; s++)
#pragma unroll
        for (int k = 0; k < 4; k++) {
            const uint32_t w = rs_wave_sum(tot[s].c[k]);
            if (lane == 0) sm[wave][4 * s + k] = w;
        }
    __syncthreads();
    if (threadIdx.x < 4 * NS) {
        uint32_t a = 0;
        for (int i = 0; i < 4; i++) a = kb::add(a, sm[i][threadIdx.x]);
        rs.host_slot[1 + threadIdx.x] = a;
    }
    asm volatile("s_waitcnt vmcnt(0)" ::: "memory");
    __syncthreads();
    if (threadIdx.x == 0) rs.host_slot[0] = seq;
}

struct RoundSyncSlot { uint32_t* d_counter; uint32_t* h_slot; };
int round_sync_acquire(RoundSyncSlot* out, hipStream_t stream);
void round_sync_release(RoundSyncSlot slot);

struct RoundSyncHost {
    uint32_t* d_counter = nullptr;
    uint32_t* h_slot = nullptr;
    uint32_t seq = 0;
    hipStream_t s = nullptr;
    int init(hipStream_t stream) {
        s = stream;
        RoundSyncSlot slot;
        SP1HIP_TRY(round_sync_acquire(&slot, stream));
        d_counter = slot.d_counter;
        h_slot = slot.h_slot;
        seq = h_slot[0];
        return SP1HIP_SUCCESS;
    }
    bool pending = false;
    ~RoundSyncHost() {
        if (d_counter && pending) (void)hipStreamSynchronize(s);
        if (d_counter) round_sync_release(RoundSyncSlot{d_counter, h_slot});
    }
    RoundSync next() { seq++; pending = true; return RoundSync{d_counter, (volatile uint32_t*)h_slot}; }
    RoundSync chained() { pending = true; return RoundSync{d_counter, nullptr}; }
    void settled() { pending = false; }
    int wait(uint32_t* out, int n_words) {
        volatile uint32_t* slot = h_slot;
        SP1HIP_TRY(wait_for_seq(slot, seq, s, "a sumcheck round result"));
        __atomic_thread_fence(__ATOMIC_ACQUIRE);
        pending = false;
        for (int k = 0; k < n_words; k++) out[k] = slot[1 + k];
        return SP1HIP_SUCCESS;
    }
};

constexpr uint32_t MAILBOX_WORDS = 16384 + 32;

int mailbox_publish(const uint32_t* d_src, uint32_t n_words, uint32_t* h_slot, uint32_t seq, hipStream_t s);

struct MailboxSlot { uint32_t* h_slot; };
int mailbox_acquire(MailboxSlot* out);
void mailbox_release(MailboxSlot slot);

struct Mailbox {
    uint32_t* h_slot = nullptr;
    uint32_t seq = 0;
    hipStream_t s = nullptr;
    int init(hipStream_t stream) {
        s = stream;
        MailboxSlot slot;
        SP1HIP_TRY(mailbox_acquire(&slot));
        h_slot = slot.h_slot;
        seq = h_slot[0];
        return SP1HIP_SUCCESS;
    }
    bool pending = false;
    ~Mailbox() {
        if (h_slot && pending) (void)hipStreamSynchronize(s);
        if (h_slot) mailbox_release(MailboxSlot{h_slot});
    }
    int fetch(const void* d_src, size_t n_words, void* out) {
        if (n_words > MAILBOX_WORDS) {
            SP1HIP_HIP(hipMemcpyAsync(out, d_src, n_words * 4, hipMemcpyDeviceToHost, s));
            SP1HIP_HIP(hipStreamSynchronize(s));
            return SP1HIP_SUCCESS;
        }
        SP1HIP_TRY(mailbox_publish((const uint32_t*)d_src, (uint32_t)n_words, h_slot, seq + 1, s));
        return wait_next(out, n_words);
    }
    int wait_next(void* out, size_t n_words, size_t first_word = 1) {
        seq++;
        pending = true;
        volatile uint32_t* slot = h_slot;
        SP1HIP_TRY(wait_for_seq(slot, seq, s, "a device result"));
        __atomic_thread_fence(__ATOMIC_ACQUIRE);
        pending = false;
        uint32_t* o = (uint32_t*)out;
        for (size_t k = 0; k < n_words; k++) o[k] = slot[first_word + k];
        return SP1HIP_SUCCESS;
    }
};

constexpr size_t PINNED_STAGE_BYTES = (size_t)2 << 20;
struct PinnedBlock { uint8_t* h; };
int pinned_stage_acquire(PinnedBlock* out);
void pinned_stage_release(PinnedBlock b);

struct PinnedStage {
    uint8_t* h = nullptr;
    size_t used = 0;
    hipStream_t s = nullptr;
    std::vector<uint8_t*> extra;
    int init(hipStream_t stream) {
        s = stream;
        PinnedBlock b;
        SP1HIP_TRY(pinned_stage_acquire(&b));
        h = b.h;
        return SP1HIP_SUCCESS;
    }
    ~PinnedStage() {
        if (h && used && hipStreamQuery(s) != hipSuccess) (void)hipStreamSynchronize(s);
        if (h) pinned_stage_release(PinnedBlock{h});
        for (uint8_t* b : extra) pinned_stage_release(PinnedBlock{b});
    }
    int upload(void* d_dst, const void* src, size_t bytes) {
        if (bytes == 0) return SP1HIP_SUCCESS;
        const size_t at = (used + 63) & ~(size_t)63;
        if (h && at + bytes <= PINNED_STAGE_BYTES) {
            memcpy(h + at, src, bytes);
            used = at + bytes;
            SP1HIP_HIP(hipMemcpyAsync(d_dst, h + at, bytes, hipMemcpyHostToDevice, s));
        } else if (h && bytes <= 16 * PINNED_STAGE_BYTES) {
            size_t off = 0;
            while (off < bytes) {
                PinnedBlock b;
                if (pinned_stage_acquire(&b) != SP1HIP_SUCCESS) break;
                extra.push_back(b.h);
                const size_t n = std::min(PINNED_STAGE_BYTES, bytes - off);
                memcpy(b.h, (const uint8_t*)src + off, n);
                SP1HIP_HIP(hipMemcpyAsync((uint8_t*)d_dst + off, b.h, n, hipMemcpyHostToDevice, s));
                off += n;
            }
            used = std::max<size_t>(used, 1);
            if (off < bytes) SP1HIP_HIP(hipMemcpyAsync((uint8_t*)d_dst + off, (const uint8_t*)src + off, bytes - off, hipMemcpyHostToDevice, s));
        } else {
            SP1HIP_HIP(hipMemcpyAsync(d_dst, src, bytes, hipMemcpyHostToDevice, s));
        }
        return SP1HIP_SUCCESS;
    }
};

}
```

Before: 97.00 million.

## Add deep GKR passes folding and summing up to four variables per launch

Adds a look-ahead planner that, when slots fit the flat layout, chooses GKR passes folding or summing three or four row variables at once instead of two. New deep kernels compute sums over a 3^k evaluation grid, and a host routine derives the k round polynomials and challenges from that grid. The aim is fewer kernel launches and host-device round-trips per layer. The cost is larger host slots and partials, more per-block reduction work, and a more complex pass schedule.

```diff
diff --git a/__graft_entry__.py b/__graft_entry__.py
--- a/__graft_entry__.py
+++ b/__graft_entry__.py
@@ -58,7 +58,8 @@
                        ("riscv_sys_rows", ["tg_riscv_sys_rows.hpp", "tg_rv64_partition.hpp", "tg_riscv_core_rows.hpp", "tg_riscv_rows.hpp", "kb31.hpp",
                                            os.path.join(ROOT, "include", "sp1hip.h")]),
                        ("lookup_counts", ["tg_lookup_counts.hpp", "kb31.hpp", os.path.join(ROOT, "include", "sp1hip.h")]),
-                       ("septic_ops", ["septic.hpp", "poseidon2.hpp", "kb_poseidon2_rc.inc", "kb31.hpp"])):
+                       ("septic_ops", ["septic.hpp", "poseidon2.hpp", "kb_poseidon2_rc.inc", "kb31.hpp"]),
+                       ("gkr_rounds", ["gkr_rounds_host.hpp", "kb31.hpp"])):
         src = os.path.join(ROOT, "tests", "native", name + ".hip")
         exe = src[:-4]
         if not os.path.exists(src):
diff --git a/sp1_amd/csrc/gkr.hip b/sp1_amd/csrc/gkr.hip
--- a/sp1_amd/csrc/gkr.hip
+++ b/sp1_amd/csrc/gkr.hip
@@ -18,6 +18,7 @@
 #include "tensor_table.hpp"
 #include "ext_host.hpp"
 #include "gkr_kernels.hpp"
+#include "gkr_rounds_host.hpp"
 
 namespace sp1hip {
 
@@ -29,7 +30,7 @@
 
 using namespace ext_host;
 
-using Poly4 = std::array<Ext, 4>;
+using gkr_rounds::Poly4;
 Ext poly_eval(const Poly4& c, const Ext& x) { return ((c[3] * x + c[2]) * x + c[1]) * x + c[0]; }
 
 Poly4 interpolate4(const Ext (&xs)[4], const Ext (&ys)[4]) {
@@ -81,6 +82,7 @@
 };
 
 constexpr uint32_t MAX_TILES = 512;
+constexpr uint64_t GKR_LOOKAHEAD_DEFAULT = 4;
 uint32_t tiles_for(uint64_t threads) { return (uint32_t)std::min<uint64_t>(std::max<uint64_t>((threads + 255) / 256, 1), MAX_TILES); }
 
 struct ParsedInt { uint32_t is_send, kind; std::vector<uint32_t> mult; std::vector<std::vector<uint32_t>> values; };
@@ -149,26 +151,58 @@
     std::vector<PassDesc> all_descs;
     std::vector<uint16_t> flat_index;
 };
-size_t count_passes(int L) { size_t n = 0; for (int v = 1; v <= L - 1; v++) n += (size_t)(v + 1) / 2 + 1; return n; }
-
-void plan_passes(const Levels& lv, uint32_t flat_max_slots, Ext* const (&scratch)[2], Ext* host_rows, PassPlan& plan) {
+struct PassChoice { int sv; bool flat; uint64_t total_slots; };
+PassChoice choose_pass(const std::vector<uint32_t>& rows_in, int fv, int left, int depth, uint32_t flat_max_slots) {
+    auto total_slots = [&](int sv) {
+        uint64_t n = 0;
+        for (uint32_t rin : rows_in) { const uint32_t ro = (rin + (1u << fv) - 1) >> fv; n += ((ro + (1u << sv) - 1) >> sv) << sv; }
+        return n;
+    };
+    const bool index_fits = rows_in.size() <= 65536;
+    if (depth > 2 && left > 2) {
+        const int sv = std::min(depth, left);
+        const uint64_t n = total_slots(sv);
+        if (n <= flat_max_slots && index_fits) return PassChoice{sv, true, n};
+    }
+    const int sv = std::min(2, left);
+    const uint64_t n = total_slots(sv);
+    return PassChoice{sv, n <= flat_max_slots && index_fits, n};
+}
+size_t count_passes(const Levels& lv, uint32_t flat_max_slots, int depth) {
+    size_t n = 0;
+    std::vector<uint32_t> rows_in(lv.K);
+    for (int v = 1; v <= lv.L - 1; v++) {
+        for (uint32_t i = 0; i < lv.K; i++) rows_in[i] = (lv.rows_at(i, v + 1) + 1) / 2;
+        for (int t = v, fv = 0;;) {
+            const int sv = choose_pass(rows_in, fv, t - fv, depth, flat_max_slots).sv;
+            for (uint32_t& r : rows_in) r = (r + (1u << fv) - 1) >> fv;
+            t -= fv;
+            n++;
+            if (sv == 0) break;
+            fv = sv;
+        }
+    }
+    return n;
+}
+
+void plan_passes(const Levels& lv, uint32_t flat_max_slots, int depth, size_t n_passes, Ext* const (&scratch)[2], Ext* host_rows, PassPlan& plan) {
     const uint32_t K = lv.K;
     auto scratch_ptr = [&](int b, uint32_t i, int which, const std::vector<size_t>& so) -> Ext* { return scratch[b] + 4 * so[i] + (size_t)which * (so[i + 1] - so[i]); };
     constexpr uint32_t TARGET_TILES = 2048;
-    plan.all_descs.reserve(count_passes(lv.L) * K);
+    plan.all_descs.reserve(n_passes * K);
     std::vector<uint32_t> rows_in(K);
     std::vector<size_t> so_prev, so_next;
     for (int v = 1; v <= lv.L - 1; v++) {
         for (uint32_t i = 0; i < K; i++) rows_in[i] = (lv.rows_at(i, v + 1) + 1) / 2;
         int cur = 0, t = v, fv = 0, pass = 0;
         for (;;) {
-            const int sv = std::min(2, t - fv);
+            const PassChoice choice = choose_pass(rows_in, fv, t - fv, depth, flat_max_slots);
+            const int sv = choice.sv;
             const bool first = pass <= 1;
             if (fv > 0) { so_next.assign(K + 1, 0); for (uint32_t i = 0; i < K; i++) so_next[i + 1] = so_next[i] + ((rows_in[i] + (1u << fv) - 1) >> fv); }
-            uint64_t total_slots = 0;
             auto slots_of = [&](uint32_t rin) -> uint32_t { const uint32_t ro = (rin + (1u << fv) - 1) >> fv; return ((ro + (1u << sv) - 1) >> sv) << sv; };
-            for (uint32_t i = 0; i < K; i++) total_slots += slots_of(rows_in[i]);
-            const bool flat = total_slots <= flat_max_slots && K <= 65536;
+            const uint64_t total_slots = choice.total_slots;
+            const bool flat = choice.flat;
             const uint32_t tile_size = flat ? 1u : (uint32_t)std::max<uint64_t>(256, ((total_slots + TARGET_TILES - 1) / TARGET_TILES + 255) / 256 * 256);
             const size_t flat_off = plan.flat_index.size();
             plan.all_descs.resize(plan.all_descs.size() + K);
@@ -187,7 +221,8 @@
                 if (flat) plan.flat_index.insert(plan.flat_index.end(), n_tiles, (uint16_t)i);
                 tile0 += n_tiles;
             }
-            if (flat) plan.shapes.push_back(PassShape{fv, sv, first, std::max<uint32_t>((tile0 + 255) / 256, 1), tile_size, tile0, flat_off, true});
+            const uint32_t wg_slots = fv > 2 ? 64 : 256;
+            if (flat) plan.shapes.push_back(PassShape{fv, sv, first, std::max<uint32_t>((tile0 + wg_slots - 1) / wg_slots, 1), tile_size, tile0, flat_off, true});
             else plan.shapes.push_back(PassShape{fv, sv, first, std::max<uint32_t>(tile0, 1), tile_size, tile0, 0, false});
             if (fv > 0) { for (uint32_t i = 0; i < K; i++) rows_in[i] = (rows_in[i] + (1u << fv) - 1) >> fv; so_prev = so_next; cur ^= 1; }
             t -= fv;
@@ -217,38 +252,6 @@
         return a;
     }
 };
-
-Poly4 eq_times_quadratic(const Ext& scale, const Ext& pt, const Ext (&q)[3]) {
-    const Ext e0 = scale * (kb::ext_one() - pt), e1 = scale * (pt + pt - kb::ext_one());
-    return Poly4{e0 * q[0], e0 * q[1] + e1 * q[0], e0 * q[2] + e1 * q[1], e1 * q[2]};
-}
-void quadratic(const Ext& g0, const Ext& g1, const Ext& gi, Ext (&q)[3]) { q[0] = g0; q[1] = g1 - g0 - gi; q[2] = gi; }
-Ext eval_quadratic(const Ext (&q)[3], const Ext& x) { return (q[2] * x + q[1]) * x + q[0]; }
-
-void row_rounds_closed_form(int sv, const Ext (&S)[10], const std::vector<Ext>& row_point, int t, Ext& PA, LayerRounds& lr, Ext& a0, Ext& a1) {
-    const Ext one = kb::ext_one(), pt_a = row_point[t - 1];
-    if (sv == 2) {
-        const Ext pt_b = row_point[t - 2];
-        const Ext corr = one - S[9];
-        Ext c0[3], c1[3], ci[3];
-        quadratic(S[0] + corr, S[1] + corr, S[4], c0);
-        quadratic(S[2] + corr, S[3] + corr, S[5], c1);
-        quadratic(S[6], S[7], S[8], ci);
-        Ext h[3];
-        for (int k = 0; k < 3; k++) h[k] = c0[k] + pt_b * (c1[k] - c0[k]);
-        a0 = lr.finish_round(eq_times_quadratic(PA, pt_a, h), pt_a, PA);
-        const Ext g0 = eval_quadratic(c0, a0), g1 = eval_quadratic(c1, a0), gi = eval_quadratic(ci, a0);
-        Ext gy[3];
-        quadratic(g0, g1, gi, gy);
-        a1 = lr.finish_round(eq_times_quadratic(PA, pt_b, gy), pt_b, PA);
-    } else {
-        const Ext corr = one - S[3];
-        Ext h[3];
-        quadratic(S[0] + corr, S[1] + corr, S[2], h);
-        a0 = lr.finish_round(eq_times_quadratic(PA, pt_a, h), pt_a, PA);
-        a1 = kb::ext_zero();
-    }
-}
 
 constexpr size_t plane_stride(size_t n) { return ((n + 15) / 16) * 16 + 16; }
 
@@ -416,6 +419,7 @@
     struct Cloned { sp1hip_challenger_t* c = nullptr; ~Cloned() { sp1hip_challenger_free(c); } } clone;
     sp1hip_challenger_t* ch = nullptr;
     uint32_t witness = 0, flat_max_slots = 0;
+    int lookahead = 2;
     Ext alpha;
     std::vector<Ext> betas;
     std::vector<uint32_t> int_chip;
@@ -521,7 +525,8 @@
         SP1HIP_TRY(lv.alloc(L, std::move(rows), s));
         timer.mark("parse + level buffers");
         flat_max_slots = (uint32_t)env_uint("SP1HIP_GKR_FLAT_SLOTS", 65536);
-        n_passes_total = count_passes(L);
+        lookahead = (int)std::min<uint64_t>(std::max<uint64_t>(env_uint("SP1HIP_GKR_LOOKAHEAD", GKR_LOOKAHEAD_DEFAULT), 2), 4);
+        n_passes_total = count_passes(lv, flat_max_slots, lookahead);
         SP1HIP_TRY(aux_stream_for(s, 2, &side, &side_ev));
         SP1HIP_TRY(d_all.alloc(std::max<size_t>(n_passes_total * K, 1) * sizeof(PassDesc), side));
         SP1HIP_TRY(d_flat.alloc((n_passes_total * (size_t)flat_max_slots + 4) * sizeof(uint16_t), side));
@@ -636,13 +641,21 @@
         for (int b = 0; b < 2; b++) SP1HIP_TRY(scratch[b].alloc(std::max<size_t>(scratch_entries, 1) * 64, s));
         direct_final = (size_t)K * 16 + 4 <= MAILBOX_WORDS;
         Ext* const scratch_ext[2] = {scratch[0].ext(), scratch[1].ext()};
-        plan_passes(lv, flat_max_slots, scratch_ext, direct_final ? reinterpret_cast<Ext*>(mb.h_slot + 4) : nullptr, plan);
+        plan_passes(lv, flat_max_slots, lookahead, n_passes_total, scratch_ext, direct_final ? reinterpret_cast<Ext*>(mb.h_slot + 4) : nullptr, plan);
         {
-            uint32_t max_tiles = 1;
-            for (auto& sh : plan.shapes) max_tiles = std::max(max_tiles, sh.tiles);
-            SP1HIP_TRY(d_partials.alloc((size_t)max_tiles * 160, s));
+            size_t bytes = 160;
+            for (auto& sh : plan.shapes) {
+                bytes = std::max(bytes, (size_t)sh.tiles * 16 * pass_sums(sh.sv));
+                SP1HIP_GKR_REQUIRE(sh.flat || (sh.fv <= 2 && sh.sv <= 2), "internal error: a deep pass that is not flat");
+            }
+            SP1HIP_TRY(d_partials.alloc(bytes, s));
         }
         timer.mark("pass descriptors planned");
+        if (timer.on) {
+            size_t deep = 0;
+            for (auto& sh : plan.shapes) deep += sh.fv > 2 || sh.sv > 2;
+            fprintf(stderr, "[sp1hip gkr] %zu passes at look-ahead %d, of which %zu deep\n", plan.shapes.size(), lookahead, deep);
+        }
         SP1HIP_GKR_REQUIRE(plan.all_descs.size() == n_passes_total * K, "internal error: pass count");
         SP1HIP_TRY(side_stage.upload(d_all.p, plan.all_descs.data(), plan.all_descs.size() * sizeof(PassDesc)));
         SP1HIP_GKR_REQUIRE(plan.flat_index.size() * sizeof(uint16_t) <= d_flat.n, "internal error: flat index size");
@@ -680,7 +693,16 @@
 #define SP1HIP_GKR_PASS(FV, SV, F, NB, FL) hipLaunchKernelGGL((gkr_pass<FV, SV, F, NB, FL>), dim3(shape.tiles), dim3(256), 0, s, d_descs, (const Ext*)d_eq_int.p, Tp, TLp, c0, c1, d_partials.u32(), rs, publish_rows ? mb.seq + 1 : rsync.seq, K, shape.tile_size, fa)
 #define SP1HIP_GKR_PASS_FL(FV, SV, F, NB) do { if (shape.flat) SP1HIP_GKR_PASS(FV, SV, F, NB, true); else SP1HIP_GKR_PASS(FV, SV, F, NB, false); } while (0)
 #define SP1HIP_GKR_PASS_SRC(FV, SV) do { if (nbase) SP1HIP_GKR_PASS_FL(FV, SV, true, true); else if (shape.first) SP1HIP_GKR_PASS_FL(FV, SV, true, false); else SP1HIP_GKR_PASS_FL(FV, SV, false, false); } while (0)
-    int launch_pass(size_t idx, int v, int t_after, const Ext& c0, const Ext& c1) {
+#define SP1HIP_GKR_DEEP_K(FV, SV, F, NB) hipLaunchKernelGGL((SP1HIP_GKR_DEEP_NAME(FV)<FV, SV, F, NB>), dim3(shape.tiles), dim3(256), 0, s, d_descs, (const Ext*)d_eq_int.p, Tp, TLp, ch, d_partials.u32(), rs, seq, fa)
+#define SP1HIP_GKR_DEEP_NAME(FV) SP1HIP_GKR_DEEP_NAME_##FV
+#define SP1HIP_GKR_DEEP_NAME_0 gkr_pass_deep
+#define SP1HIP_GKR_DEEP_NAME_2 gkr_pass_deep
+#define SP1HIP_GKR_DEEP_NAME_3 gkr_pass_deep_fold
+#define SP1HIP_GKR_DEEP_NAME_4 gkr_pass_deep_fold
+#define SP1HIP_GKR_DEEP_FIRST(FV, SV) else if (fv == FV && sv == SV) { if (nbase) SP1HIP_GKR_DEEP_K(FV, SV, true, true); else SP1HIP_GKR_DEEP_K(FV, SV, true, false); }
+#define SP1HIP_GKR_DEEP(FV, SV) else if (fv == FV && sv == SV) { if (nbase) SP1HIP_GKR_DEEP_K(FV, SV, true, true); else if (shape.first) SP1HIP_GKR_DEEP_K(FV, SV, true, false); else SP1HIP_GKR_DEEP_K(FV, SV, false, false); }
+    int launch_pass(size_t idx, int v, int t_after, const Ext (&a)[4]) {
+        const Ext &c0 = a[0], &c1 = a[1];
         const PassShape shape = plan.shapes[idx];
         const PassDesc* d_descs = (const PassDesc*)d_all.p + idx * K;
         const int fv = shape.fv, sv = shape.sv;
@@ -692,6 +714,18 @@
         const Ext* Tp = sv > 0 ? d_T.ext() + (((size_t)1 << (t_after - sv)) - 1) : (const Ext*)nullptr;
         const Ext* TLp = sv > 0 ? d_TL.ext() + (((size_t)1 << (t_after - sv)) - 1) : (const Ext*)nullptr;
         ScopedTimer tm(fv == 0 ? "gkr_pass_sum" : sv == 0 ? "gkr_pass_fold" : "gkr_pass_fold_sum", s);
+        if (fv > 2 || sv > 2) {
+            const DeepChallenges ch{{a[0], a[1], a[2], a[3]}};
+            const uint32_t seq = publish_rows ? mb.seq + 1 : rsync.seq;
+            if (false) {}
+            SP1HIP_GKR_DEEP_FIRST(0, 3) SP1HIP_GKR_DEEP_FIRST(0, 4)
+            SP1HIP_GKR_DEEP(2, 3) SP1HIP_GKR_DEEP(2, 4)
+            SP1HIP_GKR_DEEP(3, 0) SP1HIP_GKR_DEEP(3, 1) SP1HIP_GKR_DEEP(3, 2) SP1HIP_GKR_DEEP(3, 3)
+            SP1HIP_GKR_DEEP(4, 0) SP1HIP_GKR_DEEP(4, 1) SP1HIP_GKR_DEEP(4, 2) SP1HIP_GKR_DEEP(4, 3) SP1HIP_GKR_DEEP(4, 4)
+            else { set_error("internal error: GKR pass shape (%d, %d)", fv, sv); return SP1HIP_ERROR_RUNTIME; }
+            SP1HIP_LAUNCH_CHECK();
+            return SP1HIP_SUCCESS;
+        }
         if (fv == 0 && sv == 2) { if (nbase) SP1HIP_GKR_PASS_FL(0, 2, true, true); else SP1HIP_GKR_PASS_FL(0, 2, true, false); }
         else if (fv == 0 && sv == 1) { if (nbase) SP1HIP_GKR_PASS_FL(0, 1, true, true); else SP1HIP_GKR_PASS_FL(0, 1, true, false); }
         else if (fv == 2 && sv == 2) SP1HIP_GKR_PASS_SRC(2, 2);
@@ -702,6 +736,14 @@
         SP1HIP_LAUNCH_CHECK();
         return SP1HIP_SUCCESS;
     }
+#undef SP1HIP_GKR_DEEP
+#undef SP1HIP_GKR_DEEP_FIRST
+#undef SP1HIP_GKR_DEEP_K
+#undef SP1HIP_GKR_DEEP_NAME
+#undef SP1HIP_GKR_DEEP_NAME_0
+#undef SP1HIP_GKR_DEEP_NAME_2
+#undef SP1HIP_GKR_DEEP_NAME_3
+#undef SP1HIP_GKR_DEEP_NAME_4
 #undef SP1HIP_GKR_PASS_SRC
 #undef SP1HIP_GKR_PASS_FL
 #undef SP1HIP_GKR_PASS
@@ -724,31 +766,35 @@
         }
         EqTabs eq_tabs;
         Ext PA = k.one;
-        Ext a0 = k.zero, a1 = k.zero;
+        Ext a[4] = {k.zero, k.zero, k.zero, k.zero};
+        int folds = 0;
+        auto finish = [&lr](const Poly4& poly, const Ext& pt, Ext& eq_factor) { return lr.finish_round(poly, pt, eq_factor); };
         int t = v;
         for (bool first_pass = true;; first_pass = false) {
             const size_t idx = launch_idx++;
             const int fv = plan.shapes[idx].fv, sv = plan.shapes[idx].sv;
             t -= fv;
+            folds += fv > 0;
             if (!simd && t == sv) par->wake();
             timer.lap(first_pass ? GkrTimer::SKIP : GkrTimer::HOST);
-            SP1HIP_TRY(launch_pass(idx, v, t, a0, a1));
+            SP1HIP_TRY(launch_pass(idx, v, t, a));
             timer.lap(GkrTimer::LAUNCH);
             if (first_pass) eq_tabs.build(int_point, simd);
             if (sv == 0) break;
-            const int ns = sv == 2 ? 10 : 4;
-            uint32_t h_sums[40];
+            const int ns = pass_sums(sv);
+            uint32_t h_sums[4 * pass_sums(gkr_rounds::GRID_MAX_K)];
             timer.lap(GkrTimer::SKIP);
             SP1HIP_TRY(rsync.wait(h_sums, 4 * ns));
             timer.lap(GkrTimer::WAIT);
-            Ext S[10];
+            Ext S[pass_sums(gkr_rounds::GRID_MAX_K)];
             memcpy(S, h_sums, 16 * (size_t)ns);
-            row_rounds_closed_form(sv, S, row_point, t, PA, lr, a0, a1);
+            if (fv <= 2 && sv <= 2) gkr_rounds::row_rounds_closed_form(sv, S, row_point.data(), t, PA, finish, a);
+            else gkr_rounds::row_rounds_from_grid(sv, S, row_point.data(), t, PA, finish, a);
         }
         std::vector<size_t> so(K + 1, 0);
         for (uint32_t i = 0; i < K; i++) so[i + 1] = so[i] + (lv.rows_at(i, v + 1) ? 1 : 0);
         const size_t final_rows_total = so[K];
-        const int cur = (int)((((v + 1) / 2)) & 1) ^ 1;
+        const int cur = (folds - 1) & 1;
         std::vector<Ext> host(std::max<size_t>(final_rows_total, 1) * 4);
         if (direct_final) { SP1HIP_TRY(mb.wait_next(host.data(), final_rows_total * 16, 4)); rsync.pending = false; }
         else SP1HIP_TRY(mb.fetch(scratch[cur].p, final_rows_total * 16, host.data()));
diff --git a/sp1_amd/csrc/gkr_kernels.hpp b/sp1_amd/csrc/gkr_kernels.hpp
--- a/sp1_amd/csrc/gkr_kernels.hpp
+++ b/sp1_amd/csrc/gkr_kernels.hpp
@@ -490,6 +490,206 @@
     }
 }
 
+struct DeepChallenges { Ext a[4]; };
+
+template <bool FIRST, bool NBASE>
+__device__ __forceinline__ Row load_row_select(const PassDesc& d, uint32_t r) {
+    const bool live = r < d.rows_in;
+    const uint32_t rc = live ? r : d.rows_in - 1;
+    const Ext zero = kb::ext_zero(), one = kb::ext_one();
+    Row q;
+    bool live1 = live;
+    if (FIRST) {
+        const bool has1 = 2 * rc + 1 < d.rows_x;
+        const uint32_t ea = level_pos(2 * rc, d.rows_x), eb = level_pos(has1 ? 2 * rc + 1 : 2 * rc, d.rows_x);
+        q.n0 = load_n<NBASE>(d.src[0], ea); q.d0 = ld_ext((const Ext*)d.src[1], ea);
+        q.n1 = load_n<NBASE>(d.src[0], eb); q.d1 = ld_ext((const Ext*)d.src[1], eb);
+        live1 = live && has1;
+    } else {
+        const uint32_t rp = folded_pos(rc, d.rows_in);
+        q.n0 = ld_ext((const Ext*)d.src[0], rp); q.d0 = ld_ext((const Ext*)d.src[1], rp);
+        q.n1 = ld_ext((const Ext*)d.src[2], rp); q.d1 = ld_ext((const Ext*)d.src[3], rp);
+    }
+    return Row{sel_ext(live, q.n0, zero), sel_ext(live, q.d0, one), sel_ext(live1, q.n1, zero), sel_ext(live1, q.d1, one)};
+}
+
+template <int SV> struct DeepPoints {
+    uint16_t e[81];
+    constexpr DeepPoints() : e{} {
+        int n = 0, np = 1;
+        for (int j = 0; j < SV; j++) np *= 3;
+        for (int m = 0; m <= SV; m++)
+            for (int p = 0; p < np; p++) {
+                int base = 0, inf = 0, cnt = 0;
+                for (int a = 0, x = p; a < SV; a++, x /= 3) { base |= (x % 3 == 1) << a; inf |= (x % 3 == 2) << a; cnt += x % 3 == 2; }
+                if (cnt == m) e[n++] = (uint16_t)(p | base << 7 | inf << 11);
+            }
+    }
+};
+template <int SV> __device__ const DeepPoints<SV> deep_points_table{};
+
+template <int LV, bool FIRST, bool NBASE>
+__device__ __forceinline__ Row fold_rows_deep(const PassDesc& d, uint32_t r0, const DeepChallenges& ch) {
+    if constexpr (LV == 0) return load_row_select<FIRST, NBASE>(d, r0);
+    else {
+        const Row lo = fold_rows_deep<LV - 1, FIRST, NBASE>(d, r0, ch), hi = fold_rows_deep<LV - 1, FIRST, NBASE>(d, r0 + (1u << (LV - 1)), ch);
+        if constexpr (LV == 1) return lerp_row_in<NBASE>(lo, hi, ch.a[0]);
+        else return lerp_row(lo, hi, ch.a[LV - 1]);
+    }
+}
+
+constexpr int deep_points(int sv) { int n = 1; for (int j = 0; j < sv; j++) n *= 3; return n; }
+constexpr int pass_sums(int sv) { return sv == 0 ? 0 : deep_points(sv) + 1; }
+
+template <int SV, int LPR>
+__device__ __forceinline__ void deep_grid_finish(const Ext (&vals)[5], uint32_t owns, uint32_t row, bool owns_w, const Ext& w,
+                                                 uint32_t* __restrict__ partials, RoundSync rs, uint32_t seq) {
+    constexpr int CELLS = (256 / LPR) >> SV, ROWS = 1 << SV, NP = deep_points(SV), NS = NP + 1, STRIDE = CELLS + 1;
+    constexpr int STEPS = (NS * CELLS + 255) / 256;
+    static_assert(CELLS >= 1 && CELLS <= 32, "the cells of a point sit inside one wave");
+    __shared__ Ext sm_row[5][ROWS * STRIDE];
+    __shared__ Ext sm_w[CELLS];
+    __shared__ uint32_t sm_sums[4 * NS];
+    const uint32_t my = (row & (ROWS - 1u)) * STRIDE + (row >> SV);
+#pragma unroll
+    for (int t = LPR == 1 ? 1 : 0; t < 5; t++)
+        if ((owns >> t) & 1u) sm_row[t][my] = vals[t];
+    if (LPR == 1) sm_row[0][my] = vals[0];
+    if (owns_w) sm_w[row >> SV] = w;
+    __syncthreads();
+#pragma unroll
+    for (int step = 0; step < STEPS; step++) {
+        const uint32_t id = step * 256 + threadIdx.x, slot = id / CELLS, cell = id % CELLS;
+        uint32_t point = slot;
+        Ext v = kb::ext_zero();
+        if (slot < (uint32_t)NP) {
+            const uint32_t entry = deep_points_table<SV>.e[slot];
+            point = entry & 127u;
+            const uint32_t base = (entry >> 7) & 15u, inf = entry >> 11;
+            Ext gA = kb::ext_zero(), gB = gA, g0 = gA, g1 = gA;
+            uint32_t s = 0;
+            do {
+                const uint32_t at = (base | s) * STRIDE + cell;
+                const Ext rA = LPR == 1 ? sm_row[0][at] : kb::ext_add(sm_row[0][at], sm_row[1][at]);
+                if (__popc(s) & 1) { gA = kb::ext_sub(gA, rA); gB = kb::ext_sub(gB, sm_row[2][at]); g0 = kb::ext_sub(g0, sm_row[3][at]); g1 = kb::ext_sub(g1, sm_row[4][at]); }
+                else { gA = kb::ext_add(gA, rA); gB = kb::ext_add(gB, sm_row[2][at]); g0 = kb::ext_add(g0, sm_row[3][at]); g1 = kb::ext_add(g1, sm_row[4][at]); }
+                s = (s - inf) & inf;
+            } while (s != 0);
+            v = kb::ext_add(kb::ext_mul(gB, g0), kb::ext_mul(gA, g1));
+        } else if (slot == (uint32_t)NP) v = sm_w[cell];
+#pragma unroll
+        for (int off = CELLS / 2; off >= 1; off >>= 1)
+#pragma unroll
+            for (int k = 0; k < 4; k++) v.c[k] = kb::add(v.c[k], __shfl_xor(v.c[k], off, 64));
+        if (cell == 0 && slot < (uint32_t)NS)
+#pragma unroll
+            for (int k = 0; k < 4; k++) sm_sums[4 * point + k] = v.c[k];
+    }
+    __syncthreads();
+    rs_finish_block_sums<NS>(sm_sums, partials, blockIdx.x, gridDim.x, rs, seq);
+}
+
+template <int FV, int SV, bool FIRST, bool NBASE>
+__global__ __launch_bounds__(256) void gkr_pass_deep(const PassDesc* __restrict__ descs, const Ext* __restrict__ eq_int,
+                                                     const Ext* __restrict__ T, const Ext* __restrict__ TL, DeepChallenges ch,
+                                                     uint32_t* __restrict__ partials, RoundSync rs, uint32_t seq, FlatArgs fa) {
+    static_assert(FV <= 2 && SV > 2 && SV <= 4, "the two-round forms are gkr_pass, the deep folds gkr_pass_deep_fold");
+    const uint32_t p = blockIdx.x * 256 + threadIdx.x;
+    const bool valid = p < fa.total_slots;
+    const PassDesc d = descs[valid ? fa.index[p] : 0];
+    const uint32_t ro = p - d.tile0;
+    const uint32_t rows_out = (d.rows_in + (1u << FV) - 1u) >> FV;
+    Row row = padding_row();
+    if (valid && ro < rows_out) {
+        row = fold_rows_deep<FV, FIRST, NBASE>(d, ro << FV, ch);
+        if (FV > 0) {
+            const uint32_t rq = folded_pos(ro, rows_out);
+            st_ext(d.dst[0], rq, row.n0); st_ext(d.dst[1], rq, row.d0); st_ext(d.dst[2], rq, row.n1); st_ext(d.dst[3], rq, row.d1);
+        }
+    }
+    const uint32_t cells = (rows_out + (1u << SV) - 1u) >> SV, c = ro >> SV;
+    Ext w = kb::ext_zero(), wl = kb::ext_zero();
+    if (valid && c < cells) {
+        const Ext wi = ld_ext(eq_int, d.eq_int_index);
+        w = kb::ext_mul(ld_ext(T, c), wi); wl = kb::ext_mul(ld_ext(TL, c), wi);
+    }
+    constexpr bool NB = FIRST && NBASE && FV == 0;
+    const Ext A = kb::ext_add(NB ? kb::ext_mul_base(wl, row.n0.c[0]) : kb::ext_mul(row.n0, wl), kb::ext_mul(row.d0, w));
+    const Ext B = NB ? kb::ext_mul_base(wl, row.n1.c[0]) : kb::ext_mul(row.n1, wl);
+    const Ext vals[5] = {A, kb::ext_zero(), B, row.d0, row.d1};
+    deep_grid_finish<SV, 1>(vals, 0x1du, threadIdx.x, (threadIdx.x & ((1u << SV) - 1u)) == 0, w, partials, rs, seq);
+}
+
+template <int LV, bool FIRST, bool BASE>
+__device__ __forceinline__ Ext fold_table_deep(const void* src, uint32_t q, uint32_t rows_in, uint32_t rows_x, uint32_t r0,
+                                               const DeepChallenges& ch, const Ext& pad) {
+    if constexpr (LV == 0) {
+        bool live = r0 < rows_in;
+        const uint32_t rc = live ? r0 : rows_in - 1;
+        uint32_t pos;
+        if (FIRST) {
+            const uint32_t e = 2 * rc + (q >> 1);
+            const bool has = e < rows_x;
+            live = live && has;
+            pos = level_pos(has ? e : 2 * rc, rows_x);
+        } else pos = folded_pos(rc, rows_in);
+        const Ext v = BASE ? kb::ext_from_base(gptr((const uint32_t*)src)[pos]) : ld_ext((const Ext*)src, pos);
+        return sel_ext(live, v, pad);
+    } else {
+        const Ext lo = fold_table_deep<LV - 1, FIRST, BASE>(src, q, rows_in, rows_x, r0, ch, pad);
+        const Ext hi = fold_table_deep<LV - 1, FIRST, BASE>(src, q, rows_in, rows_x, r0 + (1u << (LV - 1)), ch, pad);
+        return lerp(lo, hi, ch.a[LV - 1]);
+    }
+}
+
+template <int FV, int SV, bool FIRST, bool NBASE>
+__global__ __launch_bounds__(256) void gkr_pass_deep_fold(const PassDesc* __restrict__ descs, const Ext* __restrict__ eq_int,
+                                                          const Ext* __restrict__ T, const Ext* __restrict__ TL, DeepChallenges ch,
+                                                          uint32_t* __restrict__ partials, RoundSync rs, uint32_t seq, FlatArgs fa) {
+    static_assert(FV > 2 && FV <= 4 && SV <= 4, "the shallower folds are gkr_pass and gkr_pass_deep");
+    const uint32_t q = threadIdx.x & 3u, row_wg = threadIdx.x >> 2, p = blockIdx.x * 64 + row_wg;
+    const bool valid = p < fa.total_slots;
+    const PassDesc& d = descs[valid ? fa.index[p] : 0];
+    const uint32_t rows_in = d.rows_in, ro = p - d.tile0;
+    const uint32_t rows_out = (rows_in + (1u << FV) - 1u) >> FV;
+    const Ext pad = (q & 1u) ? kb::ext_one() : kb::ext_zero();
+    Ext val = pad;
+    if (valid && ro < rows_out) {
+        const void* src = FIRST ? d.src[q & 1u] : d.src[q];
+        const uint32_t rows_x = FIRST ? d.rows_x : 0u;
+        if (FIRST && NBASE && (q & 1u) == 0) val = fold_table_deep<FV, FIRST, true>(src, q, rows_in, rows_x, ro << FV, ch, pad);
+        else val = fold_table_deep<FV, FIRST, false>(src, q, rows_in, rows_x, ro << FV, ch, pad);
+        if (SV > 0 || rs.host_slot == nullptr) st_ext(d.dst[q], folded_pos(ro, rows_out), val);
+    }
+    if constexpr (SV == 0) {
+        if (rs.host_slot != nullptr) {
+            Ext t[4];
+#pragma unroll
+            for (int u = 0; u < 4; u++)
+#pragma unroll
+                for (int k = 0; k < 4; k++) t[u].c[k] = __shfl(val.c[k], (int)((threadIdx.x & 60u) + u), 64);
+            if (q == 0 && valid && ro < rows_out) {
+                const uint32_t rq = folded_pos(ro, rows_out);
+                st_ext_host(d.dst[0], rq, t[0]); st_ext_host(d.dst[1], rq, t[1]); st_ext_host(d.dst[2], rq, t[2]); st_ext_host(d.dst[3], rq, t[3]);
+            }
+            asm volatile("s_waitcnt vmcnt(0)" ::: "memory");
+            __syncthreads();
+            if (threadIdx.x == 0 && rs_ticket_is_last_acq_rel(rs.counter, blockIdx.x, gridDim.x)) rs_publish_seq(rs.host_slot, seq);
+        }
+    } else {
+        const uint32_t cells = (rows_out + (1u << SV) - 1u) >> SV, c = ro >> SV;
+        Ext w = kb::ext_zero(), wl = kb::ext_zero();
+        if (valid && c < cells) {
+            const Ext wi = ld_ext(eq_int, d.eq_int_index);
+            w = kb::ext_mul(ld_ext(T, c), wi); wl = kb::ext_mul(ld_ext(TL, c), wi);
+        }
+        const Ext prod = q == 3 ? val : kb::ext_mul(val, q == 1 ? w : wl);
+        const Ext vals[5] = {prod, prod, prod, val, val};
+        const uint32_t owns = q == 0 ? 0x01u : q == 1 ? 0x0au : q == 2 ? 0x04u : 0x10u;
+        deep_grid_finish<SV, 4>(vals, owns, row_wg, q == 0 && (row_wg & ((1u << SV) - 1u)) == 0, w, partials, rs, seq);
+    }
+}
+
 struct OpenDesc { const uint32_t* cols; uint32_t rows, width, col0, out0; };
 constexpr int OPEN_COLS = 4, OPEN_ROWS = 16384;
 __global__ __launch_bounds__(256) void open_columns_kernel(const OpenDesc* __restrict__ descs, const uint32_t* __restrict__ eq,
diff --git a/sp1_amd/csrc/gkr_rounds_host.hpp b/sp1_amd/csrc/gkr_rounds_host.hpp
--- /dev/null
+++ b/sp1_amd/csrc/gkr_rounds_host.hpp
@@ -0,0 +1,93 @@
+#pragma once
+#include <array>
+
+#include "kb31.hpp"
+
+namespace sp1hip {
+namespace gkr_rounds {
+
+using Ext = kb::Ext;
+using Poly4 = std::array<Ext, 4>;
+
+inline Ext add(const Ext& a, const Ext& b) { return kb::ext_add(a, b); }
+inline Ext sub(const Ext& a, const Ext& b) { return kb::ext_sub(a, b); }
+inline Ext mul(const Ext& a, const Ext& b) { return kb::ext_mul(a, b); }
+
+inline Poly4 eq_times_quadratic(const Ext& scale, const Ext& pt, const Ext (&q)[3]) {
+    const Ext e0 = mul(scale, sub(kb::ext_one(), pt)), e1 = mul(scale, sub(add(pt, pt), kb::ext_one()));
+    return Poly4{mul(e0, q[0]), add(mul(e0, q[1]), mul(e1, q[0])), add(mul(e0, q[2]), mul(e1, q[1])), mul(e1, q[2])};
+}
+inline void quadratic(const Ext& g0, const Ext& g1, const Ext& gi, Ext (&q)[3]) { q[0] = g0; q[1] = sub(sub(g1, g0), gi); q[2] = gi; }
+inline Ext eval_quadratic(const Ext (&q)[3], const Ext& x) { return add(mul(add(mul(q[2], x), q[1]), x), q[0]); }
+
+template <class Finish>
+void row_rounds_closed_form(int sv, const Ext* S, const Ext* row_point, int t, Ext& PA, Finish&& finish, Ext* a) {
+    const Ext one = kb::ext_one(), pt_a = row_point[t - 1];
+    if (sv == 2) {
+        const Ext pt_b = row_point[t - 2];
+        const Ext corr = sub(one, S[9]);
+        Ext c0[3], c1[3], ci[3];
+        quadratic(add(S[0], corr), add(S[1], corr), S[4], c0);
+        quadratic(add(S[2], corr), add(S[3], corr), S[5], c1);
+        quadratic(S[6], S[7], S[8], ci);
+        Ext h[3];
+        for (int k = 0; k < 3; k++) h[k] = add(c0[k], mul(pt_b, sub(c1[k], c0[k])));
+        a[0] = finish(eq_times_quadratic(PA, pt_a, h), pt_a, PA);
+        const Ext g0 = eval_quadratic(c0, a[0]), g1 = eval_quadratic(c1, a[0]), gi = eval_quadratic(ci, a[0]);
+        Ext gy[3];
+        quadratic(g0, g1, gi, gy);
+        a[1] = finish(eq_times_quadratic(PA, pt_b, gy), pt_b, PA);
+    } else {
+        const Ext corr = sub(one, S[3]);
+        Ext h[3];
+        quadratic(add(S[0], corr), add(S[1], corr), S[2], h);
+        a[0] = finish(eq_times_quadratic(PA, pt_a, h), pt_a, PA);
+        a[1] = kb::ext_zero();
+    }
+}
+
+constexpr int GRID_MAX_K = 4;
+constexpr int grid_points(int k) { int n = 1; for (int j = 0; j < k; j++) n *= 3; return n; }
+constexpr int grid_sums(int k) { return grid_points(k) + 1; }
+
+template <class Finish>
+void row_rounds_from_grid(int k, const Ext* S, const Ext* row_point, int t, Ext& PA, Finish&& finish, Ext* a) {
+    const Ext one = kb::ext_one();
+    int n = grid_points(k);
+    Ext cur[grid_points(GRID_MAX_K)];
+    const Ext corr = sub(one, S[n]);
+    for (int g = 0; g < n; g++) {
+        bool finite = true;
+        for (int x = g, j = 0; j < k; j++, x /= 3) finite = finite && x % 3 != 2;
+        cur[g] = finite ? add(S[g], corr) : S[g];
+    }
+    for (int j = 0; j < k; j++) {
+        const Ext pt = row_point[t - 1 - j];
+        const int later = k - 1 - j;
+        Ext h[3] = {kb::ext_zero(), kb::ext_zero(), kb::ext_zero()};
+        for (int b = 0; b < (1 << later); b++) {
+            Ext wgt = one;
+            int idx = 0;
+            for (int m = 0, p3 = 1; m < later; m++, p3 *= 3) {
+                const Ext& pm = row_point[t - 2 - j - m];
+                const bool bit = (b >> m) & 1;
+                wgt = later == 0 ? wgt : mul(wgt, bit ? pm : sub(one, pm));
+                idx += bit ? p3 : 0;
+            }
+            for (int d = 0; d < 3; d++) h[d] = add(h[d], later == 0 ? cur[d] : mul(wgt, cur[3 * idx + d]));
+        }
+        Ext q[3];
+        quadratic(h[0], h[1], h[2], q);
+        a[j] = finish(eq_times_quadratic(PA, pt, q), pt, PA);
+        n /= 3;
+        for (int m = 0; m < n; m++) {
+            Ext qm[3];
+            quadratic(cur[3 * m], cur[3 * m + 1], cur[3 * m + 2], qm);
+            cur[m] = eval_quadratic(qm, a[j]);
+        }
+    }
+    for (int j = k; j < GRID_MAX_K; j++) a[j] = kb::ext_zero();
+}
+
+}
+}
diff --git a/sp1_amd/csrc/round_sync.hpp b/sp1_amd/csrc/round_sync.hpp
--- a/sp1_amd/csrc/round_sync.hpp
+++ b/sp1_amd/csrc/round_sync.hpp
@@ -20,7 +20,7 @@
 
 constexpr uint32_t RS_GROUPS = 32, RS_GROUP_STRIDE = 64;
 constexpr size_t RS_COUNTER_BYTES = (size_t)(RS_GROUPS + 1) * RS_GROUP_STRIDE * 4;
-constexpr size_t RS_SLOT_WORDS = 64;
+constexpr size_t RS_SLOT_WORDS = 512;
 
 __device__ __forceinline__ bool rs_ticket_is_last(uint32_t* counter, uint32_t block_linear, uint32_t total_blocks) {
     const uint32_t g = block_linear % RS_GROUPS, members = (total_blocks - g + RS_GROUPS - 1) / RS_GROUPS;
@@ -106,6 +106,48 @@
         for (int i = 0; i < 4; i++) a = kb::add(a, sm[i][threadIdx.x]);
         rs.host_slot[1 + threadIdx.x] = a;
     }
+    asm volatile("s_waitcnt vmcnt(0)" ::: "memory");
+    __syncthreads();
+    if (threadIdx.x == 0) rs.host_slot[0] = seq;
+}
+
+template <int NS>
+__device__ __forceinline__ void rs_finish_block_sums(const uint32_t* sums, uint32_t* __restrict__ partials, uint32_t block_linear,
+                                                     uint32_t total_blocks, RoundSync rs, uint32_t seq) {
+    constexpr int NW = 4 * NS, PER = (NW + 63) / 64;
+    static_assert(1 + NW <= (int)RS_SLOT_WORDS, "the host slot holds the sequence number and every sum");
+    __shared__ uint32_t sm[4][PER * 64];
+    __shared__ uint32_t last_flag;
+    const int lane = threadIdx.x & 63, wave = threadIdx.x >> 6;
+    for (int w = threadIdx.x; w < NW; w += 256) rs_store_partial(&partials[(size_t)block_linear * NW + w], sums[w]);
+    asm volatile("s_waitcnt vmcnt(0)" ::: "memory");
+    __syncthreads();
+    if (threadIdx.x == 0) last_flag = rs_ticket_is_last(rs.counter, block_linear, total_blocks);
+    __syncthreads();
+    if (!last_flag) return;
+    uint32_t acc[PER];
+#pragma unroll
+    for (int q = 0; q < PER; q++) acc[q] = 0;
+    constexpr uint32_t BATCH = 8;
+    for (uint32_t b0 = wave; b0 < total_blocks; b0 += 4 * BATCH) {
+        uint32_t v[BATCH][PER];
+#pragma unroll
+        for (uint32_t u = 0; u < BATCH; u++)
+#pragma unroll
+            for (int q = 0; q < PER; q++) {
+                const uint32_t b = b0 + 4 * u;
+                v[u][q] = b < total_blocks && q * 64 + lane < NW
+                    ? __hip_atomic_load(partials + (size_t)b * NW + q * 64 + lane, __ATOMIC_RELAXED, __HIP_MEMORY_SCOPE_AGENT) : 0u;
+            }
+#pragma unroll
+        for (uint32_t u = 0; u < BATCH; u++)
+#pragma unroll
+            for (int q = 0; q < PER; q++) acc[q] = kb::add(acc[q], v[u][q]);
+    }
+#pragma unroll
+    for (int q = 0; q < PER; q++) sm[wave][q * 64 + lane] = acc[q];
+    __syncthreads();
+    for (int w = threadIdx.x; w < NW; w += 256) rs.host_slot[1 + w] = kb::add(kb::add(sm[0][w], sm[1][w]), kb::add(sm[2][w], sm[3][w]));
     asm volatile("s_waitcnt vmcnt(0)" ::: "memory");
     __syncthreads();
     if (threadIdx.x == 0) rs.host_slot[0] = seq;
```

Result: faster. 99.90 million, median of 6 (+3.0%).
